# qope/starky-bn254

Measured on AMD Instinct MI355X. Metric: G1 scalar-mult proofs/sec at trace height 2^16, higher is better.
Workload: dtype u64

## Files before the change

starky_bn254_amd/csrc/kernels.cuh:

```cuda
#pragma once
#include "poseidon.cuh"
#include "air.cuh"

#include "kernels_ntt.cuh"

__global__ void pow_table_kernel(u64* out, size_t n, u64 base) {
  size_t i = (size_t)blockIdx.x * blockDim.x + threadIdx.x;
  if (i < n) out[i] = f_pow(F(base), i).v;
}
__global__ void shift_odd_table_kernel(u64* out, size_t n, const u64* __restrict__ shift, const u64* __restrict__ tw, u32 log_s) {
  size_t i = (size_t)blockIdx.x * blockDim.x + threadIdx.x;
  if (i < n) out[i] = (F(shift[i]) * F(tw[(i >> log_s) << log_s])).v;
}
__global__ void scale_pow_kernel(u64* v, size_t n, u64 base) {
  size_t i = (size_t)blockIdx.x * blockDim.x + threadIdx.x;
  if (i < n) v[i] = (F(v[i]) * f_pow(F(base), i)).v;
}

__global__ __launch_bounds__(256) __attribute__((amdgpu_waves_per_eu(4))) void leaf_hash_kernel(const u64* __restrict__ lde, size_t m, u32 lde_log, u32 ncols,
                                                        u64* __restrict__ digests) {
  size_t row = (size_t)blockIdx.x * blockDim.x + threadIdx.x;
  if (row >= m) return;
  F s[12];
#pragma unroll
  for (int i = 0; i < 12; i++) s[i] = F(0);
  size_t leaf = bitrev32((u32)row, lde_log);
  if (ncols <= 4) {
    for (u32 c = 0; c < 4; c++) digests[leaf * 4 + c] = c < ncols ? lde[(size_t)c * m + row] : 0;
    return;
  }
  for (u32 c = 0; c < ncols; c += 8) {
#pragma unroll
    for (u32 i = 0; i < 8; i++)
      if (c + i < ncols) s[i] = F(lde[(size_t)(c + i) * m + row]);
    poseidon_permute_keep(s, c + 8 >= ncols ? P_KEEP_DIGEST : (c + 16 <= ncols ? P_KEEP_CAPACITY : P_KEEP_ALL));
  }
#pragma unroll
  for (int i = 0; i < 4; i++) digests[leaf * 4 + i] = s[i].v;
}

__global__ __launch_bounds__(256) void merkle_level_kernel(const u64* __restrict__ child, u64* __restrict__ parent, size_t nparent) {
  size_t i = (size_t)blockIdx.x * blockDim.x + threadIdx.x;
  if (i >= nparent) return;
  F s[12];
#pragma unroll
  for (int k = 0; k < 8; k++) s[k] = F(child[i * 8 + k]);
#pragma unroll
  for (int k = 8; k < 12; k++) s[k] = F(0);
  poseidon_permute_keep(s, P_KEEP_DIGEST);
#pragma unroll
  for (int k = 0; k < 4; k++) parent[i * 4 + k] = s[k].v;
}

__global__ __launch_bounds__(256) __attribute__((amdgpu_waves_per_eu(4))) void leaf_absorb_kernel(const u64* __restrict__ lde_chunk, size_t m, u32 lde_log, u32 ncols_chunk,
                                                          u64* __restrict__ state, int first, int last, u64* __restrict__ digests, int next_full) {
  size_t row = (size_t)blockIdx.x * blockDim.x + threadIdx.x;
  if (row >= m) return;
  F s[12];
#pragma unroll
  for (int i = 0; i < 12; i++) s[i] = F(0);
  if (!first) {
#pragma unroll
    for (int i = 8; i < 12; i++) s[i] = F(state[(size_t)i * m + row]);
    if (ncols_chunk < 8) {
#pragma unroll
      for (int i = 0; i < 8; i++) s[i] = F(state[(size_t)i * m + row]);
    }
  }
  for (u32 c = 0; c < ncols_chunk; c += 8) {
#pragma unroll
    for (u32 i = 0; i < 8; i++)
      if (c + i < ncols_chunk) s[i] = F(lde_chunk[(size_t)(c + i) * m + row]);
    const bool end = c + 8 >= ncols_chunk;
    const int keep = end ? (last ? P_KEEP_DIGEST : (next_full ? P_KEEP_CAPACITY : P_KEEP_ALL)) : (c + 16 <= ncols_chunk ? P_KEEP_CAPACITY : P_KEEP_ALL);
    poseidon_permute_keep(s, keep);
  }
  u32 tid = threadIdx.x;
  asm volatile("" : "+v"(tid));
  const size_t row2 = (size_t)blockIdx.x * blockDim.x + tid;
  if (last) {
    size_t leaf = bitrev32((u32)row2, lde_log);
#pragma unroll
    for (int i = 0; i < 4; i++) digests[leaf * 4 + i] = s[i].v;
  } else {
#pragma unroll
    for (int i = 8; i < 12; i++) state[(size_t)i * m + row2] = s[i].v;
    if (!next_full) {
#pragma unroll
      for (int i = 0; i < 8; i++) state[(size_t)i * m + row2] = s[i].v;
    }
  }
}

static constexpr u32 MERKLE_SUBTREE_THREADS = 256;
__global__ __launch_bounds__(MERKLE_SUBTREE_THREADS) void merkle_subtree_kernel(u64* __restrict__ tree, size_t nleaf, u32 l0, u32 nlev, u32 nchild) {
  __shared__ u64 buf[2 * 256 * 4];
  const u32 tid = threadIdx.x, nt = blockDim.x;
  const u64* child = tree + (2 * nleaf - ((2 * nleaf) >> l0)) * 4;
  size_t base = (size_t)blockIdx.x * nchild;
  for (u32 e = tid; e < nchild * 4; e += nt) buf[e] = child[base * 4 + e];
  __syncthreads();
  u32 active = nchild / 2;
  const u32 groups = nt / 16, grp = tid / 16, lane = tid & 15;
  for (u32 lv = 1; lv <= nlev; lv++) {
    u64* out = tree + (2 * nleaf - ((2 * nleaf) >> (l0 + lv))) * 4;
    const size_t idx0 = ((size_t)blockIdx.x * nchild) >> lv;
    if (active > 4 * groups) {
      F s[12];
      if (tid < active) {
#pragma unroll
        for (int k = 0; k < 8; k++) s[k] = F(buf[tid * 8 + k]);
#pragma unroll
        for (int k = 8; k < 12; k++) s[k] = F(0);
        poseidon_permute_keep(s, P_KEEP_DIGEST);
      }
      __syncthreads();
      if (tid < active) {
#pragma unroll
        for (int k = 0; k < 4; k++) { buf[tid * 4 + k] = s[k].v; out[(idx0 + tid) * 4 + k] = s[k].v; }
      }
      __syncthreads();
    } else {
      u64 res[4];
      u32 nit = (active + groups - 1) / groups;
      for (u32 it = 0; it < nit; it++) {
        u32 parent = it * groups + grp;
        if (it * groups + (tid / 64) * 4 >= active) break;
        const u32 e = lane < 12 ? lane : lane - 12;
        u64 v = (parent < active && e < 8) ? buf[parent * 8 + e] : 0;
        res[it] = poseidon_permute_coop16(v, lane);
      }
      __syncthreads();
      for (u32 it = 0; it < nit; it++) {
        u32 parent = it * groups + grp;
        if (parent < active && lane < 4) { buf[parent * 4 + lane] = res[it]; out[(idx0 + parent) * 4 + lane] = res[it]; }
      }
      __syncthreads();
    }
    active >>= 1;
  }
}

__global__ __launch_bounds__(256) void merkle_level_thread_kernel(u64* __restrict__ tree, size_t nleaf, u32 l) {
  const size_t parents = nleaf >> (l + 1);
  const size_t i = (size_t)blockIdx.x * blockDim.x + threadIdx.x;
  if (i >= parents) return;
  const u64* child = tree + (2 * nleaf - ((2 * nleaf) >> l)) * 4;
  u64* out = tree + (2 * nleaf - ((2 * nleaf) >> (l + 1))) * 4;
  F s[12];
#pragma unroll
  for (int k = 0; k < 8; k++) s[k] = F(child[i * 8 + k]);
#pragma unroll
  for (int k = 8; k < 12; k++) s[k] = F(0);
  poseidon_permute_keep(s, P_KEEP_DIGEST);
#pragma unroll
  for (int k = 0; k < 4; k++) out[i * 4 + k] = s[k].v;
}
__global__ __launch_bounds__(256) void merkle_level_coop_kernel(u64* __restrict__ tree, size_t nleaf, u32 l) {
  const size_t parents = nleaf >> (l + 1);
  const size_t parent = ((size_t)blockIdx.x * blockDim.x + threadIdx.x) >> 4;
  const u32 lane = threadIdx.x & 15, e = lane < 12 ? lane : lane - 12;
  const u64* child = tree + (2 * nleaf - ((2 * nleaf) >> l)) * 4;
  u64* out = tree + (2 * nleaf - ((2 * nleaf) >> (l + 1))) * 4;
  const u64 v = (parent < parents && e < 8) ? child[parent * 8 + e] : 0;
  const u64 r = poseidon_permute_coop16(v, lane);
  if (parent < parents && lane < 4) out[parent * 4 + lane] = r;
}

__global__ __launch_bounds__(256) void fri_leaf_hash_kernel(const u64* __restrict__ va, const u64* __restrict__ vb, u32 log_m, u32 arity_bits,
// ... 202 lines not shown
  } else if (KIND == 11) {
    if (PART == 0) flag_u64_eval(cs, row, FlagU64Shape(p.num_io));
  } else if (KIND == 7 || KIND == 8) {
    const OpShape sh(KIND);
    if (PART == 0) op_eval<KIND>(cs, row, sh);
    else if (PART == 2) {
      if (seg == 2) permutation_checks(cs, row, zrow, sh, p.num_zs, F(p.gamma0), F(p.gamma1), 0, p.zsplit);
      else permutation_checks(cs, row, zrow, sh, p.num_zs, F(p.gamma0), F(p.gamma1), p.zsplit, p.num_zs);
    }
  } else {
    constexpr int E = KIND == 4 ? 12 : (KIND == 6 ? 13 : (KIND == 3 ? 2 : (KIND == 5 ? 0 : 1)));
    ExpShape sh(E, p.num_io);
    const bool moved = (E == 0 || E == 1 || E == 2) && p.lookups_in_perm;
    if (PART < 2) exp_eval<E>(cs, row, sh, (const ExpPiConsts<F>*)pic_arg, (PART == 1 && moved) ? 3 : 1 + PART);
    else {
      const int z0 = seg == 2 ? 0 : p.zsplit, z1 = seg == 2 ? p.zsplit : p.num_zs;
      permutation_checks(cs, row, zrow, sh, p.num_zs, F(p.gamma0), F(p.gamma1), z0, z1);
      if (moved) lookups_beside_permutation(cs, row, sh, p.num_zs, (z0 + 1) / 2, (z1 + 1) / 2);
    }
  }
#pragma unroll
  for (int j = 0; j < SBN_NCH; j++) p.part[((size_t)seg * SBN_NCH + j) * p.m + i] = cs.result(j).v;
}
__global__ __launch_bounds__(256) void quotient_combine_kernel(QuotientParams p) {
  size_t i = (size_t)blockIdx.x * blockDim.x + threadIdx.x;
  if (i >= p.m) return;
  F dinv(p.zh_inv[((i << p.row_shift) | p.row_rho) & 1]);
#pragma unroll
  for (int j = 0; j < SBN_NCH; j++) {
    F acc(p.part[((size_t)(QSEG - 1) * SBN_NCH + j) * p.m + i]);
#pragma unroll
    for (u32 sgm = 0; sgm + 1 < QSEG; sgm++) acc += F(p.part[((size_t)sgm * SBN_NCH + j) * p.m + i]) * F(p.seg_shift[sgm][j]);
    p.qout[(size_t)j * p.m + i] = (acc * dinv).v;
  }
}

__global__ void domain_tables_kernel(u64* xs, u64* lag_first, u64* lag_last, size_t m, u32 lde_log, u32 degree_bits) {
  size_t i = (size_t)blockIdx.x * blockDim.x + threadIdx.x;
  if (i >= m) return;
  F w = f_root_of_unity(lde_log);
  F x = F(GL_GEN) * f_pow(w, i);
  F g = f_root_of_unity(degree_bits);
  F nn = F((u64)1 << degree_bits);
  F zx = f_exp_pow2(x, degree_bits) - F(1);
  xs[i] = x.v;
  lag_first[i] = (zx * f_inv(nn * (x - F(1)))).v;
  lag_last[i] = (zx * f_inv(nn * (g * x - F(1)))).v;
}

__device__ __forceinline__ F wave_scan_mul_rev(F x, int lane) {
#pragma unroll
  for (int d = 1; d < 64; d <<= 1) {
    u64 o = __shfl_down((unsigned long long)x.v, d, 64);
    if (lane + d < 64) x = x * F(o);
  }
  return x;
}
template <int PZ_E>
__global__ __launch_bounds__(256) void permz_chunk_products_kernel(const u64* __restrict__ trace, size_t n, const PairCols* __restrict__ pairs, u64 gamma0, u64 gamma1,
                                                                   u64* __restrict__ tot) {
  __shared__ u64 wn[4], wd[4];
  const int z = blockIdx.y;
  const size_t c = blockIdx.x, chunks = gridDim.x;
  const int tid = threadIdx.x, lane = tid & 63, wv = tid >> 6;
  const size_t i0 = c * 256 * PZ_E + (size_t)tid * PZ_E;
  const u64* lhs = trace + (size_t)pairs[z].lhs * n + i0;
  const u64* rhs = trace + (size_t)pairs[z].rhs * n + i0;
  const F g0(gamma0), g1(gamma1);
  u64 lv[PZ_E], rv[PZ_E];
#pragma unroll
  for (int e = 0; e < PZ_E; e++) { lv[e] = lhs[e]; rv[e] = rhs[e]; }
  F pn(1), pd(1);
#pragma unroll
  for (int e = 0; e < PZ_E; e++) { const F l(lv[e]), r(rv[e]); pn = pn * ((l + g0) * (l + g1)); pd = pd * ((r + g0) * (r + g1)); }
#pragma unroll
  for (int d = 32; d >= 1; d >>= 1) { pn = pn * F(__shfl_xor((unsigned long long)pn.v, d, 64)); pd = pd * F(__shfl_xor((unsigned long long)pd.v, d, 64)); }
  if (lane == 0) { wn[wv] = pn.v; wd[wv] = pd.v; }
  __syncthreads();
  if (tid == 0) {
    tot[((size_t)z * chunks + c) * 2] = (F(wn[0]) * F(wn[1]) * F(wn[2]) * F(wn[3])).v;
    tot[((size_t)z * chunks + c) * 2 + 1] = (F(wd[0]) * F(wd[1]) * F(wd[2]) * F(wd[3])).v;
  }
}
__global__ __launch_bounds__(64) void permz_chunk_scan_kernel(const u64* __restrict__ tot, u32 chunks, u64* __restrict__ pq) {
  const int z = blockIdx.x, lane = threadIdx.x;
  const u64* t = tot + (size_t)z * chunks * 2;
  u64* o = pq + (size_t)z * chunks * 2;
  F carry(1), all(1);
  for (u32 b = 0; b < chunks; b += 64) {
    const u32 idx = b + lane;
    const bool on = idx < chunks;
    const F inc = wave_scan_mul(on ? F(t[2 * idx]) : F(1), lane);
    const u64 pv = __shfl_up((unsigned long long)inc.v, 1, 64);
    if (on) o[2 * idx] = (lane == 0 ? carry : carry * F(pv)).v;
    carry = carry * F(__shfl((unsigned long long)inc.v, 63, 64));
    F d = on ? F(t[2 * idx + 1]) : F(1);
#pragma unroll
    for (int k = 32; k >= 1; k >>= 1) d = d * F(__shfl_xor((unsigned long long)d.v, k, 64));
    all = all * d;
  }
  F carry_s = f_inv(all);
  for (u32 b = ((chunks - 1) / 64) * 64;; b -= 64) {
    const u32 idx = b + lane;
    const bool on = idx < chunks;
    const F inc = wave_scan_mul_rev(on ? F(t[2 * idx + 1]) : F(1), lane);
    const u64 sv = __shfl_down((unsigned long long)inc.v, 1, 64);
    if (on) o[2 * idx + 1] = (lane == 63 ? carry_s : carry_s * F(sv)).v;
    carry_s = carry_s * F(__shfl((unsigned long long)inc.v, 0, 64));
    if (b == 0) break;
  }
}
template <int PZ_E>
__global__ __launch_bounds__(256) void permz_chunk_write_kernel(const u64* __restrict__ trace, size_t n, const PairCols* __restrict__ pairs, u64 gamma0, u64 gamma1,
                                                                const u64* __restrict__ pq, u64* __restrict__ zout) {
  __shared__ u64 wn[4], wd[4];
  const int z = blockIdx.y;
  const size_t c = blockIdx.x, chunks = gridDim.x;
  const int tid = threadIdx.x, lane = tid & 63, wv = tid >> 6;
  const size_t i0 = c * 256 * PZ_E + (size_t)tid * PZ_E;
  const u64* lhs = trace + (size_t)pairs[z].lhs * n + i0;
  const u64* rhs = trace + (size_t)pairs[z].rhs * n + i0;
  u64* zc = zout + (size_t)z * n + i0;
  const F g0(gamma0), g1(gamma1);
  u64 lv[PZ_E], rv[PZ_E];
#pragma unroll
  for (int e = 0; e < PZ_E; e++) { lv[e] = lhs[e]; rv[e] = rhs[e]; }
  F pn[PZ_E], sd[PZ_E];
#pragma unroll
  for (int e = 0; e < PZ_E; e++) { const F l(lv[e]); const F num = (l + g0) * (l + g1); pn[e] = e ? pn[e - 1] * num : num; }
#pragma unroll
  for (int e = PZ_E - 1; e >= 0; e--) { const F r(rv[e]); const F den = (r + g0) * (r + g1); sd[e] = e < PZ_E - 1 ? sd[e + 1] * den : den; }
  const F incn = wave_scan_mul(pn[PZ_E - 1], lane), incd = wave_scan_mul_rev(sd[0], lane);
  if (lane == 63) wn[wv] = incn.v;
  if (lane == 0) wd[wv] = incd.v;
  __syncthreads();
  F pre(pq[((size_t)z * chunks + c) * 2]), suf(pq[((size_t)z * chunks + c) * 2 + 1]);
  for (int w = 0; w < wv; w++) pre = pre * F(wn[w]);
  for (int w = 3; w > wv; w--) suf = suf * F(wd[w]);
  const u64 pv = __shfl_up((unsigned long long)incn.v, 1, 64), sv = __shfl_down((unsigned long long)incd.v, 1, 64);
  const F exn = lane == 0 ? pre : pre * F(pv);
  const F exd = lane == 63 ? suf : suf * F(sv);
  const F both = exn * exd;
  zc[0] = (both * sd[0]).v;
#pragma unroll
  for (int e = 1; e < PZ_E; e++) zc[e] = (both * pn[e - 1] * sd[e]).v;
}

__global__ void ext_pow_table_kernel(u64* pa, u64* pb, size_t n, u64 z0, u64 z1) {
  size_t i = (size_t)blockIdx.x * blockDim.x + threadIdx.x;
  if (i >= n) return;
  E2 r = e2_pow(E2(F(z0), F(z1)), i);
  pa[i] = r.a.v; pb[i] = r.b.v;
}
__device__ __forceinline__ F block_sum(F v, u64* sh) {
  const int lane = threadIdx.x & 63, wv = threadIdx.x >> 6;
#pragma unroll
  for (int d = 32; d >= 1; d >>= 1) v = v + F(__shfl_xor((unsigned long long)v.v, d, 64));
  __syncthreads();
  if (lane == 0) sh[wv] = v.v;
  __syncthreads();
  F t(0);
  for (unsigned w = 0; w < blockDim.x / 64; w++) t = t + F(sh[w]);
  return t;
}
template <u32 OPEN_UNROLL>
__global__ __launch_bounds__(256) void openings_kernel(const u64* __restrict__ coeffs, size_t n, const u64* __restrict__ pa0, const u64* __restrict__ pb0,
                                                       const u64* __restrict__ pa1, const u64* __restrict__ pb1, u64* __restrict__ out) {
  __shared__ u64 sh[4];
  const u64* c = coeffs + (size_t)blockIdx.x * n;
  Acc<F> s0, r0, s1, r1;
  s0.clear(); r0.clear(); s1.clear(); r1.clear();
  for (size_t i = threadIdx.x; i < n; i += 256 * OPEN_UNROLL) {
    u64 cv[OPEN_UNROLL], t0[OPEN_UNROLL], t1[OPEN_UNROLL], t2[OPEN_UNROLL], t3[OPEN_UNROLL];
#pragma unroll
    for (u32 k = 0; k < OPEN_UNROLL; k++) {
      const size_t ik = i + 256 * k;
      cv[k] = c[ik]; t0[k] = pa0[ik]; t1[k] = pb0[ik]; t2[k] = pa1[ik]; t3[k] = pb1[ik];
    }
    __builtin_amdgcn_sched_barrier(0);
#pragma unroll
    for (u32 k = 0; k < OPEN_UNROLL; k++) {
      const F v{cv[k]};
      s0.macv(v, F(t0[k])); r0.macv(v, F(t1[k]));
      s1.macv(v, F(t2[k])); r1.macv(v, F(t3[k]));
    }
  }
  const F a0 = block_sum(s0.value(), sh), b0 = block_sum(r0.value(), sh), a1 = block_sum(s1.value(), sh), b1 = block_sum(r1.value(), sh);
  if (threadIdx.x == 0) {
    u64* o = out + (size_t)blockIdx.x * 4;
    o[0] = a0.v; o[1] = b0.v; o[2] = a1.v; o[3] = b1.v;
  }
}

template <u32 OPEN_UNROLL>
__global__ __launch_bounds__(256) void openings1_kernel(const u64* __restrict__ coeffs, size_t n, const u64* __restrict__ pa, const u64* __restrict__ pb,
                                                        u64* __restrict__ out, u32 off) {
  __shared__ u64 sh[4];
  const u64* c = coeffs + (size_t)blockIdx.x * n;
  Acc<F> s0, r0;
  s0.clear(); r0.clear();
  for (size_t i = threadIdx.x; i < n; i += 256 * OPEN_UNROLL) {
    u64 cv[OPEN_UNROLL], t0[OPEN_UNROLL], t1[OPEN_UNROLL];
#pragma unroll
    for (u32 k = 0; k < OPEN_UNROLL; k++) {
      const size_t ik = i + 256 * k;
      cv[k] = c[ik]; t0[k] = pa[ik]; t1[k] = pb[ik];
    }
    __builtin_amdgcn_sched_barrier(0);
#pragma unroll
    for (u32 k = 0; k < OPEN_UNROLL; k++) {
      const F v{cv[k]};
      s0.macv(v, F(t0[k])); r0.macv(v, F(t1[k]));
    }
  }
  const F a0 = block_sum(s0.value(), sh), b0 = block_sum(r0.value(), sh);
  if (threadIdx.x == 0) {
    u64* o = out + (size_t)blockIdx.x * 4 + off;
    o[0] = a0.v; o[1] = b0.v;
  }
}

__global__ __launch_bounds__(256) void fri_combine_partial_kernel(const u64* __restrict__ coeffs, size_t n, u32 npoly, u32 group_size,
                                                                  const u64* __restrict__ pa, const u64* __restrict__ pb, u64* __restrict__ part_a,
                                                                  u64* __restrict__ part_b) {
  size_t i = (size_t)blockIdx.x * blockDim.x + threadIdx.x;
  if (i >= n) return;
  const u32 g = blockIdx.y;
  const u32 j0 = g * group_size, cnt = j0 + group_size < npoly ? group_size : npoly - j0;
  const u64* c = coeffs + (size_t)j0 * n + i;
  Acc<F> a, b;
  a.clear(); b.clear();
  u32 k = 0;
  for (; k + 8 <= cnt; k += 8) {
    u64 f[8];
#pragma unroll
    for (u32 u = 0; u < 8; u++) f[u] = c[(size_t)(k + u) * n];
#pragma unroll
    for (u32 u = 0; u < 8; u++) { const F v(f[u]); a.mac(v, F(pa[k + u])); b.mac(v, F(pb[k + u])); }
  }
  for (; k < cnt; k++) { const F v(c[(size_t)k * n]); a.mac(v, F(pa[k])); b.mac(v, F(pb[k])); }
  part_a[(size_t)g * n + i] = a.value().v; part_b[(size_t)g * n + i] = b.value().v;
}
__global__ void fri_combine_reduce_kernel(const u64* part_a, const u64* part_b, size_t n, u32 ngroups, const u64* w, u64* out_a, u64* out_b, int accumulate) {
  size_t i = (size_t)blockIdx.x * blockDim.x + threadIdx.x;
  if (i >= n) return;
  E2 acc = accumulate ? E2(F(out_a[i]), F(out_b[i])) : E2(F(0), F(0));
  for (u32 g = 0; g < ngroups; g++) acc += E2(F(part_a[(size_t)g * n + i]), F(part_b[(size_t)g * n + i])) * E2(F(w[2 * g]), F(w[2 * g + 1]));
  out_a[i] = acc.a.v; out_b[i] = acc.b.v;
}

static constexpr u32 DBL_CHUNK = 16;
__global__ __launch_bounds__(256) void divide_by_linear_pass1(const u64* __restrict__ ca, const u64* __restrict__ cb, size_t nchunks, u64 z0, u64 z1,
                                                              u64* __restrict__ ha, u64* __restrict__ hb) {
  const size_t t = (size_t)blockIdx.x * blockDim.x + threadIdx.x;
  if (t >= nchunks) return;
  const E2 z{F(z0), F(z1)};
  const size_t s = t * DBL_CHUNK;
  E2 h{F(0), F(0)};
  for (u32 k = DBL_CHUNK; k-- > 0;) h = h * z + E2(F(ca[s + k]), F(cb[s + k]));
  ha[t] = h.a.v; hb[t] = h.b.v;
}
template <u32 U> __device__ __forceinline__ void dbl_fold(const u64* ha, const u64* hb, size_t base, size_t per, const E2 zl, E2& g) {
  for (size_t j0 = per; j0 > 0; j0 -= U) {
    u64 va[U], vb[U];
#pragma unroll
    for (u32 k = 0; k < U; k++) { va[k] = ha[base + j0 - 1 - k]; vb[k] = hb[base + j0 - 1 - k]; }
#pragma unroll
    for (u32 k = 0; k < U; k++) g = E2(F(va[k]), F(vb[k])) + zl * g;
  }
}
template <u32 U> __device__ __forceinline__ void dbl_replay(u64* ha, u64* hb, size_t base, size_t per, const E2 zl, E2 carry) {
  for (size_t j0 = per; j0 > 0; j0 -= U) {
    u64 va[U], vb[U];
#pragma unroll
    for (u32 k = 0; k < U; k++) { va[k] = ha[base + j0 - 1 - k]; vb[k] = hb[base + j0 - 1 - k]; }
#pragma unroll
    for (u32 k = 0; k < U; k++) {
      ha[base + j0 - 1 - k] = carry.a.v; hb[base + j0 - 1 - k] = carry.b.v;
      carry = E2(F(va[k]), F(vb[k])) + zl * carry;
    }
  }
}
__global__ __launch_bounds__(256) void divide_by_linear_pass2(u64* __restrict__ ha, u64* __restrict__ hb, size_t nchunks, u64 z0, u64 z1) {
  __shared__ u64 sa[2][256], sb[2][256];
  const int tid = threadIdx.x;
  const int lanes = nchunks < 256 ? (int)nchunks : 256;
  const size_t per = nchunks / lanes, base = (size_t)tid * per;
  const bool live = tid < lanes;
  const E2 zl = e2_pow(E2{F(z0), F(z1)}, DBL_CHUNK);
  E2 g{F(0), F(0)};
  if (live) { if (per % 8 == 0) dbl_fold<8>(ha, hb, base, per, zl, g); else dbl_fold<1>(ha, hb, base, per, zl, g); }
  E2 m = e2_pow(zl, per);
  int cur = 0;
  sa[0][tid] = g.a.v; sb[0][tid] = g.b.v;
  __syncthreads();
  for (int d = 1; d < lanes; d <<= 1) {
    E2 v{F(sa[cur][tid]), F(sb[cur][tid])};
    if (tid + d < lanes) v = v + m * E2(F(sa[cur][tid + d]), F(sb[cur][tid + d]));
    sa[cur ^ 1][tid] = v.a.v; sb[cur ^ 1][tid] = v.b.v;
    m = m * m;
    cur ^= 1;
    __syncthreads();
  }
  E2 carry{F(0), F(0)};
  if (tid + 1 < lanes) carry = E2(F(sa[cur][tid + 1]), F(sb[cur][tid + 1]));
  if (live) { if (per % 8 == 0) dbl_replay<8>(ha, hb, base, per, zl, carry); else dbl_replay<1>(ha, hb, base, per, zl, carry); }
}
__global__ __launch_bounds__(256) void divide_by_linear_pass3(const u64* __restrict__ ca, const u64* __restrict__ cb, size_t nchunks, u64 z0, u64 z1,
                                                              const u64* __restrict__ ha, const u64* __restrict__ hb, u64 mul0, u64 mul1,
                                                              u64* __restrict__ oa, u64* __restrict__ ob, int accumulate, u32 times_x) {
  const size_t t = (size_t)blockIdx.x * blockDim.x + threadIdx.x;
  if (t >= nchunks) return;
  const E2 z{F(z0), F(z1)}, mul{F(mul0), F(mul1)};
  const size_t s = t * DBL_CHUNK, n = nchunks * DBL_CHUNK;
  E2 b{F(ha[t]), F(hb[t])};
  for (u32 k = DBL_CHUNK; k-- > 0;) {
    const size_t i = s + k;
    const E2 q = b;
    b = b * z + E2(F(ca[i]), F(cb[i]));
    const size_t j = i + times_x;
    if (j >= n) continue;
    const E2 o = accumulate ? E2(F(oa[j]), F(ob[j])) * mul + q : q;
    oa[j] = o.a.v; ob[j] = o.b.v;
  }
}

__global__ void fri_fold_kernel(const u64* ca, const u64* cb, size_t nout, u32 arity, u64 b0, u64 b1, u64* oa, u64* ob) {
  size_t i = (size_t)blockIdx.x * blockDim.x + threadIdx.x;
  if (i >= nout) return;
  E2 beta{F(b0), F(b1)}, acc(F(0), F(0));
  for (u32 t = arity; t-- > 0;) acc = acc * beta + E2(F(ca[i * arity + t]), F(cb[i * arity + t]));
  oa[i] = acc.a.v; ob[i] = acc.b.v;
}

struct PowParams { u64 state[12]; u32 wpos; u32 min_lz; u64 base; u64 count; u64* result; };
__global__ __launch_bounds__(256) void pow_kernel(PowParams p) {
  u64 gid = (u64)blockIdx.x * blockDim.x + threadIdx.x;
  if (gid >= p.count) return;
  F s[12];
#pragma unroll
  for (int i = 0; i < 12; i++) s[i] = F(p.state[i]);
  s[p.wpos] = F(p.base + gid);
  poseidon_permute(s);
  u64 resp = s[P_RATE - 1].v;
  u32 lz = resp ? (u32)__clzll((long long)resp) : 64;
  if (lz >= p.min_lz) atomicMin((unsigned long long*)p.result, (unsigned long long)(p.base + gid));
}

__global__ __launch_bounds__(256) void split_pack_kernel(const u64* __restrict__ lde, size_t m, u32 nc, u32 ob, u32 log_r, u32 me,
                                                         u64* __restrict__ send_l, u64* __restrict__ send_n, u64* __restrict__ self_l, u64* __restrict__ self_n) {
  const size_t i = (size_t)blockIdx.x * blockDim.x + threadIdx.x;
  const u32 c = blockIdx.y;
  if (i >= m || c >= nc) return;
  const u64 v = lde[(size_t)c * m + i];
  const size_t ml = m >> log_r, rmask = ((size_t)1 << log_r) - 1;
  const u32 s = bitrev32((u32)(i & rmask), log_r);
  if (s == me) self_l[(size_t)c * ml + (i >> log_r)] = v;
  else send_l[((size_t)s * ob + c) * ml + (i >> log_r)] = v;
  if (send_n) {
    const size_t p = (i + m - 2) & (m - 1);
    const u32 s2 = bitrev32((u32)(p & rmask), log_r);
    if (s2 == me) self_n[(size_t)c * ml + (p >> log_r)] = v;
    else send_n[((size_t)s2 * ob + c) * ml + (p >> log_r)] = v;
  }
}
__global__ void split_unpack_rows_kernel(const u64* __restrict__ in, size_t m, u32 nplanes, u32 log_r, u64* __restrict__ out) {
  const size_t i = (size_t)blockIdx.x * blockDim.x + threadIdx.x;
  if (i >= m) return;
  const size_t ml = m >> log_r;
  const u32 s = bitrev32((u32)(i & (((size_t)1 << log_r) - 1)), log_r);
  for (u32 p = 0; p < nplanes; p++) out[(size_t)p * m + i] = in[((size_t)s * nplanes + p) * ml + (i >> log_r)];
// ... 36 lines not shown
```

starky_bn254_amd/csrc/poseidon.cuh:

```cuda
#pragma once
#include "gl.cuh"
#include "settings.hpp"
#include <utility>

static constexpr int P_WIDTH = 12;
static constexpr int P_RATE = 8;
enum { P_KEEP_ALL = 0, P_KEEP_CAPACITY = 1, P_KEEP_DIGEST = 2 };

static const u64 POSEIDON_RC_HOST[360] = {
#include "poseidon_consts.inc"
};
static __constant__ u64 POSEIDON_RC_DEV[360] = {
#include "poseidon_consts.inc"
};

static const u64 POSEIDON_EFF_HOST[360] = {
#include "poseidon_eff_consts.inc"
};
static __constant__ u64 POSEIDON_EFF_DEV[360] = {
#include "poseidon_eff_consts.inc"
};

static __constant__ u64 POSEIDON_KX_DEV[8 * 24] = {
#include "poseidon_kx_consts.inc"
// ... 226 lines not shown
}
__device__ __forceinline__ void mds3(u64* s, u64 d1, u64 d2, u64 tb) {
  u32 lo[12], hi[12];
#pragma unroll
  for (int i = 0; i < 12; i++) { lo[i] = (u32)s[i]; hi[i] = (u32)(s[i] >> 32); }
  u64 al[12], ah[12];
  mds3_half(lo, (u32)d1, (u32)d2, al, tb);
  mds3_half(hi, (u32)(d1 >> 32), (u32)(d2 >> 32), ah, tb);
#pragma unroll
  for (int r = 0; r < 12; r += 3) fold3(al + r, ah + r, s + r);
}
}

__device__ __forceinline__ void poseidon_permute_fast(F* st, int keep = P_KEEP_ALL) {
  u64 rcb = (u64)POSEIDON_EFF_DEV, tb = (u64)pw::MDS_FUSED_TABLE, kxb = (u64)POSEIDON_KX_DEV;
  asm volatile("" : "+s"(rcb), "+s"(tb), "+s"(kxb));
  typedef const __attribute__((address_space(4))) u64* cptr;
  const cptr rc = (cptr)rcb;
  const pw::kx_ptr kx = (pw::kx_ptr)kxb;
  u64 s[12];
#pragma unroll
  for (int i = 0; i < 12; i++) s[i] = pw::add_c(st[i].v, rc[i]);
  int r = 4;
#pragma unroll 1
  for (int k = 0; k < 4; k++) {
    u32 lo[12], hi[12];
#pragma unroll
    for (int i = 0; i < 12; i += 3) pw::sbox3(s[i], s[i + 1], s[i + 2], lo + i, hi + i);
    pw::mdsc(lo, hi, s, kx + 24 * k);
  }
#pragma unroll 1
  for (int k = 0; k < 6; k++, r += 3) {
    s[0] = pw::sbox(pw::add_c(s[0], rc[12 * r]));
    const u64 y0p = pw::sbox(pw::add_c(pw::mds_row0(s), rc[12 * (r + 1)]));
    const u64 z0p = pw::sbox(pw::add_c(pw::mds2_row0(s, y0p, tb), rc[12 * (r + 2)]));
    pw::mds3(s, y0p, z0p, tb);
  }
#pragma unroll 1
  for (int k = 0; k < 2; k++, r += 2) {
    s[0] = pw::sbox(pw::add_c(s[0], rc[12 * r]));
    pw::mds2(s, pw::sbox(pw::add_c(pw::mds_row0(s), rc[12 * (r + 1)])), tb);
  }
#pragma unroll
  for (int i = 0; i < 12; i++) s[i] = pw::add_c(s[i], rc[12 * 26 + i]);
#pragma unroll 1
  for (int k = 4; k < 7; k++) {
    u32 lo[12], hi[12];
#pragma unroll
    for (int i = 0; i < 12; i += 3) pw::sbox3(s[i], s[i + 1], s[i + 2], lo + i, hi + i);
    pw::mdsc(lo, hi, s, kx + 24 * k);
  }
  {
    u32 lo[12], hi[12];
#pragma unroll
    for (int i = 0; i < 12; i += 3) pw::sbox3(s[i], s[i + 1], s[i + 2], lo + i, hi + i);
    if (keep == P_KEEP_CAPACITY) {
      pw::mdsq<8>(lo, hi, s + 8);
#pragma unroll
      for (int i = 8; i < 12; i++) st[i] = F(gp::canon(s[i]));
    } else if (keep == P_KEEP_DIGEST) {
      pw::mdsq<0>(lo, hi, s);
#pragma unroll
      for (int i = 0; i < 4; i++) st[i] = F(gp::canon(s[i]));
    } else {
      pw::mds(lo, hi, s);
#pragma unroll
      for (int i = 0; i < 12; i++) st[i] = F(gp::canon(s[i]));
    }
  }
}
namespace pc {
template <int I> __device__ __forceinline__ u32 rot(u32 x, bool use2) {
  const u32 y1 = (u32)__builtin_amdgcn_update_dpp(0, (int)x, 0x120 + (16 - I), 0xf, 0xf, false);
  const u32 y2 = (u32)__builtin_amdgcn_update_dpp(0, (int)x, 0x120 + (12 - I), 0xf, 0xf, false);
  return use2 ? y2 : y1;
}
template <int I> __device__ __forceinline__ void term(u32 lo, u32 hi, u32 lane16, u64& al, u64& ah) {
  constexpr u32 C[12] = {17, 15, 41, 16, 2, 28, 13, 13, 39, 18, 34, 20};
  if constexpr (I == 0) { al += (u64)lo * C[0]; ah += (u64)hi * C[0]; }
  else {
    const bool use2 = lane16 >= 12 || lane16 + I >= 16;
    al += (u64)rot<I>(lo, use2) * C[I]; ah += (u64)rot<I>(hi, use2) * C[I];
  }
}
template <int... I> __device__ __forceinline__ void mds_row(u32 lo, u32 hi, u32 lane16, u64& al, u64& ah, std::integer_sequence<int, I...>) {
  (term<I>(lo, hi, lane16, al, ah), ...);
}
}
__device__ __forceinline__ u64 poseidon_permute_coop16(u64 v, u32 lane) {
  const u64* rc = POSEIDON_EFF_DEV;
  const u32 lane16 = lane & 15, j = lane16 < 12 ? lane16 : lane16 - 12;
  for (int r = 0; r < 30; r++) {
    v = pw::add_c(v, rc[12 * r + j]);
    const bool full = r < 4 || r >= 26;
    u64 sb = pw::sbox(v);
    v = (full || j == 0) ? sb : v;
    u32 lo = (u32)v, hi = (u32)(v >> 32);
    u64 al = 0, ah = 0;
    pc::mds_row(lo, hi, lane16, al, ah, std::make_integer_sequence<int, 12>{});
    if (j == 0) { al += (u64)lo * 8u; ah += (u64)hi * 8u; }
    u32 h0 = (u32)ah, h1 = (u32)(ah >> 32);
    u64 t = al + ((u64)h0 << 32);
    u32 c = t < al;
    u64 add = (u64)(h1 + c) * GLEPS;
    u64 o = t + add;
    if (o < add) o += GLEPS;
    v = o;
  }
  return v >= GLP ? v - GLP : v;
}
#else
__device__ u64 poseidon_permute_coop16(u64 v, u32 lane);
#endif

#if !defined(__HIP_DEVICE_COMPILE__)
#include "poseidon_fast_consts.inc"
namespace ph {
typedef unsigned __int128 u128;
struct Acc { u128 lo = 0, hi = 0; };
static inline void mac(Acc& a, u64 x, u64 y) { u128 p = (u128)x * y; a.lo += (u64)p; a.hi += (u64)(p >> 64); }
static inline u64 fold(const Acc& a) {
  u128 t = a.lo + a.hi * (u128)GLEPS;
  return gl_reduce128((u64)t, (u64)(t >> 64));
}
}
#if defined(__x86_64__)
#include <immintrin.h>
#include <cstdlib>
#define PH_AVX512 __attribute__((target("avx512f,avx512dq")))
PH_AVX512 static inline __m512i mulred_x8(__m512i a, __m512i b) {
  const __m512i M32 = _mm512_set1_epi64(0xFFFFFFFFLL);
  const __m512i ah = _mm512_srli_epi64(a, 32), bh = _mm512_srli_epi64(b, 32);
  const __m512i ll = _mm512_mul_epu32(a, b), lh = _mm512_mul_epu32(a, bh), hl = _mm512_mul_epu32(ah, b), hh = _mm512_mul_epu32(ah, bh);
  const __m512i mid = _mm512_add_epi64(lh, _mm512_srli_epi64(ll, 32));
  const __m512i mid2 = _mm512_add_epi64(hl, _mm512_and_si512(mid, M32));
  const __m512i lo = _mm512_or_si512(_mm512_and_si512(ll, M32), _mm512_slli_epi64(mid2, 32));
  const __m512i hi = _mm512_add_epi64(hh, _mm512_add_epi64(_mm512_srli_epi64(mid, 32), _mm512_srli_epi64(mid2, 32)));
  const __m512i hi_hi = _mm512_srli_epi64(hi, 32), hi_lo = _mm512_and_si512(hi, M32);
  const __mmask8 bw = _mm512_cmplt_epu64_mask(lo, hi_hi);
  __m512i t0 = _mm512_sub_epi64(lo, hi_hi);
  t0 = _mm512_mask_sub_epi64(t0, bw, t0, M32);
  const __m512i t1 = _mm512_sub_epi64(_mm512_slli_epi64(hi_lo, 32), hi_lo);
  __m512i r = _mm512_add_epi64(t0, t1);
  const __mmask8 cy = _mm512_cmplt_epu64_mask(r, t1);
  return _mm512_mask_add_epi64(r, cy, r, M32);
}
PH_AVX512 static inline __m512i sbox7_x8(__m512i x, __m512i c) {
  const __m512i M32 = _mm512_set1_epi64(0xFFFFFFFFLL);
  __m512i y = _mm512_add_epi64(x, c);
  y = _mm512_mask_add_epi64(y, _mm512_cmplt_epu64_mask(y, c), y, M32);
  const __m512i y2 = mulred_x8(y, y), y4 = mulred_x8(y2, y2), y3 = mulred_x8(y2, y);
  return mulred_x8(y4, y3);
}
PH_AVX512 static void full_round_sboxes_avx512(u64* s, const u64* rc) {
  const __m512i a = sbox7_x8(_mm512_loadu_si512(s), _mm512_loadu_si512(rc));
  const __m512i b = sbox7_x8(_mm512_maskz_loadu_epi64(0x0F, s + 8), _mm512_maskz_loadu_epi64(0x0F, rc + 8));
  _mm512_storeu_si512(s, a);
  _mm512_mask_storeu_epi64(s + 8, 0x0F, b);
}
PH_AVX512 static inline void mds_x12(__m512i& A, __m512i& B) {
  static const u64 C[12] = {17, 15, 41, 16, 2, 28, 13, 13, 39, 18, 34, 20};
  const __m512i M32 = _mm512_set1_epi64(0xFFFFFFFFLL);
  const __m512i lane = _mm512_set_epi64(7, 6, 5, 4, 3, 2, 1, 0);
  const __m512i twelve = _mm512_set1_epi64(12);
  __m512i slA = _mm512_setzero_si512(), shA = slA, slB = slA, shB = slA;
#pragma GCC unroll 12
  for (int i = 0; i < 12; i++) {
    __m512i ia = _mm512_add_epi64(lane, _mm512_set1_epi64(i));
    ia = _mm512_mask_sub_epi64(ia, _mm512_cmpge_epu64_mask(ia, twelve), ia, twelve);
    __m512i ib = _mm512_add_epi64(lane, _mm512_set1_epi64((i + 8) % 12));
    ib = _mm512_mask_sub_epi64(ib, _mm512_cmpge_epu64_mask(ib, twelve), ib, twelve);
    const __m512i xa = _mm512_permutex2var_epi64(A, ia, B), xb = _mm512_permutex2var_epi64(A, ib, B);
    const __m512i ca = i == 0 ? _mm512_set_epi64(17, 17, 17, 17, 17, 17, 17, 25) : _mm512_set1_epi64((long long)C[i]);
    const __m512i cb = _mm512_set1_epi64((long long)C[i]);
    slA = _mm512_add_epi64(slA, _mm512_mul_epu32(xa, ca)); shA = _mm512_add_epi64(shA, _mm512_mul_epu32(_mm512_srli_epi64(xa, 32), ca));
    slB = _mm512_add_epi64(slB, _mm512_mul_epu32(xb, cb)); shB = _mm512_add_epi64(shB, _mm512_mul_epu32(_mm512_srli_epi64(xb, 32), cb));
  }
  auto fold = [&](__m512i sl, __m512i sh) PH_AVX512 {
    const __m512i shl = _mm512_slli_epi64(sh, 32);
    const __m512i l = _mm512_add_epi64(sl, shl);
    const __m512i one = _mm512_set1_epi64(1);
    __m512i h = _mm512_srli_epi64(sh, 32);
    h = _mm512_mask_add_epi64(h, _mm512_cmplt_epu64_mask(l, shl), h, one);
    const __m512i t1 = _mm512_sub_epi64(_mm512_slli_epi64(h, 32), h);
    const __m512i r = _mm512_add_epi64(l, t1);
    return _mm512_mask_add_epi64(r, _mm512_cmplt_epu64_mask(r, t1), r, M32);
  };
  A = fold(slA, shA); B = fold(slB, shB);
}
PH_AVX512 static void full_rounds_x4_avx512(u64* s, const u64* rc) {
  __m512i A = _mm512_loadu_si512(s), B = _mm512_maskz_loadu_epi64(0x0F, s + 8);
  for (int k = 0; k < 4; k++) {
    A = sbox7_x8(A, _mm512_loadu_si512(rc + 12 * k));
    B = sbox7_x8(B, _mm512_maskz_loadu_epi64(0x0F, rc + 12 * k + 8));
    mds_x12(A, B);
  }
  const __m512i P = _mm512_set1_epi64((long long)GLP);
  A = _mm512_mask_sub_epi64(A, _mm512_cmpge_epu64_mask(A, P), A, P);
  B = _mm512_mask_sub_epi64(B, _mm512_cmpge_epu64_mask(B, P), B, P);
  _mm512_storeu_si512(s, A);
  _mm512_mask_storeu_epi64(s + 8, 0x0F, B);
}
static inline bool host_has_avx512() {
  static const bool have = __builtin_cpu_supports("avx512f") && __builtin_cpu_supports("avx512dq") && !sbn::Settings::from_env_or_default().no_avx512;
  return have;
}
#endif
static inline void full_rounds_host(F* s, const u64* rc, int& r) {
#if defined(__x86_64__)
  if (host_has_avx512()) {
    static_assert(sizeof(F) == sizeof(u64), "F is one u64");
    full_rounds_x4_avx512(reinterpret_cast<u64*>(s), rc + 12 * r);
    r += 4;
    return;
  }
#endif
  for (int k = 0; k < 4; k++, r++) {
    for (int i = 0; i < 12; i++) s[i] = sbox7(s[i] + F(rc[12 * r + i]));
    poseidon_mds(s);
  }
}
struct PartialChainTables { u64 PI[22][11]; u64 K[22][22]; };
static inline const PartialChainTables& partial_chain_tables() {
  static const PartialChainTables T = [] {
    PartialChainTables t{};
    for (int k = 0; k < 22; k++) {
      for (int j = 0; j < 11; j++) { F acc(0); for (int i = 0; i < 11; i++) acc = acc + F(PFAST_VHAT[11 * k + i]) * F(PFAST_INIT[11 * i + j]); t.PI[k][j] = acc.v; }
      for (int q = 0; q < k; q++) { F acc(0); for (int i = 0; i < 11; i++) acc = acc + F(PFAST_VHAT[11 * k + i]) * F(PFAST_WHAT[11 * q + i]); t.K[k][q] = acc.v; }
    }
    return t;
  }();
  return T;
}
static inline void poseidon_permute_host_fast(F* s) {
  const u64* rc = POSEIDON_EFF_HOST;
  int r = 0;
  full_rounds_host(s, rc, r);
  for (int i = 0; i < 12; i++) s[i] = s[i] + F(rc[12 * r + i]);
  const PartialChainTables& T = partial_chain_tables();
  u64 u[11], t[22];
  for (int i = 0; i < 11; i++) u[i] = s[1 + i].v;
  ph::Acc fin[11];
  for (int i = 0; i < 11; i++) for (int j = 0; j < 11; j++) ph::mac(fin[i], PFAST_INIT[11 * i + j], u[j]);
  ph::Acc nxt; for (int j = 0; j < 11; j++) ph::mac(nxt, T.PI[0][j], u[j]);
  u64 cur = s[0].v;
  for (int k = 0; k < 22; k++, r++) {
    t[k] = sbox7(k ? F(cur) + F(rc[12 * r]) : F(cur)).v;
    ph::Acc a = nxt;
    for (int q = 0; q < k; q++) ph::mac(a, T.K[k][q], t[q]);
    ph::mac(a, PFAST_M00, t[k]);
    cur = ph::fold(a);
    nxt = ph::Acc();
    if (k + 1 < 22) for (int j = 0; j < 11; j++) ph::mac(nxt, T.PI[k + 1][j], u[j]);
    for (int i = 0; i < 11; i++) ph::mac(fin[i], PFAST_WHAT[11 * k + i], t[k]);
  }
  s[0] = F(cur);
  for (int i = 0; i < 11; i++) s[1 + i] = F(ph::fold(fin[i]));
  full_rounds_host(s, rc, r);
}
#endif

GL_HD void poseidon_permute(F* s) {
#if defined(__HIP_DEVICE_COMPILE__)
  poseidon_permute_fast(s);
#else
  poseidon_permute_host_fast(s);
#endif
}
GL_HD void poseidon_permute_keep(F* s, int keep) {
#if defined(__HIP_DEVICE_COMPILE__)
  poseidon_permute_fast(s, keep);
#else
  (void)keep;
  poseidon_permute_host_fast(s);
#endif
}

struct Digest4 { F e[4]; };

GL_HD Digest4 poseidon_two_to_one(const Digest4& l, const Digest4& r) {
  F s[12];
#pragma unroll
  for (int i = 0; i < 4; i++) { s[i] = l.e[i]; s[4 + i] = r.e[i]; s[8 + i] = F(0); }
  poseidon_permute(s);
  Digest4 d;
#pragma unroll
  for (int i = 0; i < 4; i++) d.e[i] = s[i];
  return d;
}
```

starky_bn254_amd/csrc/prover.hip:

```cpp
#include "host_common.hpp"
#include "settings.hpp"
#include "kernels.cuh"
#include "kernels_tracegen.cuh"
#include <algorithm>
#include <cstring>
#include <cstdlib>
#include <thread>
#include <atomic>
#include <chrono>

using namespace sbn;

namespace sbn { thread_local std::string g_last_error; }

#define HIPC(expr)                                                                                   \
  do {                                                                                               \
    hipError_t e_ = (expr);                                                                          \
    if (e_ != hipSuccess) return fail(SBN_ERR_HIP, "%s failed: %s (%s:%d)", #expr, hipGetErrorString(e_), __FILE__, __LINE__); \
  } while (0)

static std::atomic<int> g_default_device{0};
static thread_local int t_device = -1;
static inline int cur_device() { return t_device >= 0 ? t_device : g_default_device.load(); }
#define g_device (cur_device())
namespace sbn { int current_device() { return cur_device(); } }

enum Stage {
  ST_TRACE_COMMIT, ST_PERM_Z, ST_Z_COMMIT, ST_QUOTIENT_EVAL, ST_QUOTIENT_COMMIT,
  ST_OPENINGS, ST_FRI_COMBINE, ST_FRI_LAYERS, ST_POW, ST_QUERIES, ST_COUNT
};
enum Extra { EX_TRACE_ABSORB_MS, EX_TRACE_ABSORB_LAUNCHES, EX_Z_ABSORB_MS, EX_Z_ABSORB_LAUNCHES, EX_TRACEGEN_MS, EX_COMM_MS, EX_COUNT };
static const char* STAGE_NAMES[ST_COUNT + EX_COUNT] = {
  "trace_commit", "perm_z", "z_commit", "quotient_eval", "quotient_commit",
  "openings", "fri_combine", "fri_layers", "pow", "queries",
  "trace_absorb_kernels_ms", "trace_absorb_launches", "z_absorb_kernels_ms", "z_absorb_launches", "device_tracegen_ms",
  "split_exchange_ms"};
static constexpr int MAX_CHUNKS = 512;

struct DevTree {
  u64* d = nullptr; size_t nleaf = 0; u32 nlevels = 0;
  u64* level(u32 l) const { return d + (2 * nleaf - ((2 * nleaf) >> l)) * 4; }
};

struct ColShare {
  size_t total = 0, ob = 64; u32 R = 1, rank = 0;
  size_t nblocks() const { return (total + ob - 1) / ob; }
  size_t steps() const { return (nblocks() + R - 1) / R; }
  size_t block_cols(size_t b) const { return b < nblocks() ? std::min(ob, total - b * ob) : 0; }
  size_t own_cols(u32 r) const { size_t s = 0; for (size_t b = r; b < nblocks(); b += R) s += block_cols(b); return s; }
  size_t own() const { return own_cols(rank); }
  size_t max_own() const { size_t s = 0; for (u32 r = 0; r < R; r++) s = std::max(s, own_cols(r)); return s; }
  size_t global_col(u32 r, size_t local) const { return ((local / ob) * R + r) * ob + local % ob; }
};
struct SplitCtx {
  sbn_comm comm;
  u32 log_r = 0, rho = 0;
  size_t ml = 0;
  ColShare cs, zs;
  size_t cr = 0, zr = 0;
  u32 planes = 1;
  u64 *lde_l = nullptr, *lde_n = nullptr, *zlde_l = nullptr, *zlde_n = nullptr, *scratch = nullptr;
  size_t scratch_words = 0;
  size_t slot_words = 0;
  u64* d_ldechunk = nullptr;
  u32* d_idx_local = nullptr;
  PairCols* d_pairs_own = nullptr;
  hipStream_t cstream = nullptr;
  hipEvent_t xchg_done[MAX_CHUNKS];
  std::vector<hipEvent_t> tev;
  size_t tev_used = 0;
};

struct sbn_prover {
  AirShape air; sbn_config cfg; FriShape fri;
  SplitCtx* sp = nullptr;
  size_t lde_scratch_words = 0;
  u32 degree_bits, lde_log; size_t n, m;
  int device; hipStream_t stream;
  u64 *d_trace = nullptr, *d_coef = nullptr, *d_lde = nullptr, *d_tmp = nullptr;
  u64 *d_zval = nullptr, *d_zcoef = nullptr, *d_zlde = nullptr;
  u64 *d_q = nullptr, *d_qlde = nullptr;
  DevTree tree_t, tree_z, tree_q;
  std::vector<DevTree> fri_trees;
  u64 *d_tw_f = nullptr, *d_tw_i = nullptr, *d_shift = nullptr, *d_shift_inv = nullptr;
  u64 *d_shift_odd = nullptr;
  u64 *d_xs = nullptr, *d_lag_first = nullptr, *d_lag_last = nullptr;
  u64 *d_apow = nullptr;
  size_t apow_n = 0;
  void* d_pic = nullptr;
  PairCols* d_pairs = nullptr;
  u64 *d_zpow = nullptr;
  u64 *d_open = nullptr;
  u64 *d_part = nullptr;
  u64 *d_w = nullptr;
  u64 *d_fa = nullptr, *d_fb = nullptr;
  u64 *d_fcoef = nullptr;
  u64 *d_fcoef2 = nullptr;
  std::vector<u64*> fri_vals;
  u64 *d_pow = nullptr;
  u32 *d_idx = nullptr;
  u64 *d_qbuf = nullptr; size_t qstride = 0;
  std::vector<u64> pi;
  bool loaded = false;
  hipEvent_t ev[ST_COUNT + 1];
  float stage_ms[ST_COUNT + EX_COUNT];
  size_t ntt_chunk;
  size_t ntt_sub = 0;
  bool ntt_xcd = true;
  bool fast_ntt = true;
  bool ntt_fused = false;
  u64* d_tmp2 = nullptr;
  hipStream_t rstream = nullptr;
  hipEvent_t rows_done = nullptr, rc_done = nullptr;
  int* d_rc_err = nullptr;
  bool rc_pending = false;
  size_t rc_first_col = 0;
  u64* d_tmp3 = nullptr;
  bool ntt_fused512 = false;
  hipStream_t hstream = nullptr;
  hipStream_t nstream = nullptr;
  hipEvent_t intt_done[MAX_CHUNKS];
  bool ntt_two_streams = false;
  Settings set;
  unsigned gen_calls = 0;
  int chain_mode = 0;
  hipEvent_t chunk_ready[MAX_CHUNKS];
  hipEvent_t abs_ev[2 * MAX_CHUNKS];
  hipEvent_t hash_done;
  u64* d_sponge = nullptr;
  u64* h_chain = nullptr;
  size_t h_chain_words = 0;
  u64* h_io = nullptr;
  size_t h_io_words = 0;
  u64* h_open = nullptr;
  u64* h_open2 = nullptr;
};

static int dmalloc(u64** p, size_t words) {
  HIPC(hipMalloc((void**)p, words * sizeof(u64)));
  return 0;
}

static u32 pick_log_t(u32 log_r, u32 log_s) {
  u32 lt = 4;
  while (lt > 0 && ((size_t)(1u << log_r) * ((1u << lt) + 1) * 8) > 48 * 1024) lt--;
  return std::min(lt, log_s);
}
static int ntt_columns(sbn_prover* P, const u64* in, size_t in_cs, u64* out, size_t out_cs, u64* tmp, size_t tmp_cs, size_t ncols,
                       u32 log_n, bool inverse, size_t n_in, const u64* pre, const u64* post, u64 scale, hipStream_t st = nullptr, int which = 3) {
  if (ncols == 0) return 0;
  if (!st) st = P->stream;
  u32 log_n1 = (log_n + 1) / 2, log_n2 = log_n - log_n1;
  size_t n1 = (size_t)1 << log_n1, n2 = (size_t)1 << log_n2;
  NttPassParams a{};
  a.in = in; a.out = tmp; a.in_col_stride = in_cs; a.out_col_stride = tmp_cs;
  a.log_r = log_n1; a.log_t = pick_log_t(log_n1, log_n2); a.log_n = log_n;
  a.in_sr = n2; a.in_st = 1; a.out_sr = n2; a.out_st = 1; a.n_in = n_in;
  a.r_fast_load = 0; a.twiddle = 1; a.tw = inverse ? P->d_tw_i : P->d_tw_f; a.tw_log = P->lde_log;
  a.pre = pre; a.post = nullptr; a.scale = 1;
  NttPassParams b{};
  b.in = tmp; b.out = out; b.in_col_stride = tmp_cs; b.out_col_stride = out_cs;
  b.log_r = log_n2; b.log_t = pick_log_t(log_n2, log_n1); b.log_n = log_n;
  b.in_sr = 1; b.in_st = n2; b.out_sr = n1; b.out_st = 1; b.n_in = (size_t)1 << log_n;
  b.r_fast_load = 1; b.twiddle = 0; b.tw = a.tw; b.tw_log = P->lde_log;
  b.pre = nullptr; b.post = post; b.scale = scale;
  for (size_t c0 = 0; c0 < ncols; c0 += 32768) {
    size_t nc = std::min<size_t>(32768, ncols - c0);
    NttPassParams pa = a, pb = b;
    pa.in = a.in + c0 * in_cs; pa.out = a.out + c0 * tmp_cs;
    pb.in = b.in + c0 * tmp_cs; pb.out = b.out + c0 * out_cs;
    dim3 ga((unsigned)(n2 >> pa.log_t), (unsigned)nc), gb((unsigned)(n1 >> pb.log_t), (unsigned)nc);
    size_t la = ((size_t)1 << pa.log_r) * ((1u << pa.log_t) + 1) * 8, lb = ((size_t)1 << pb.log_r) * ((1u << pb.log_t) + 1) * 8;
    const u32 kperm = inverse ? 11u : 5u;
    auto launch = [&](NttPassParams q, dim3 grid, size_t lds_bytes) {
      const bool fast = P->fast_ntt && q.log_t == 4 && (q.log_r == 8 || q.log_r == 9);
      if (fast && P->ntt_xcd) { q.xcd_order = 1; std::swap(grid.x, grid.y); }
      if (fast && q.log_r == 8) hipLaunchKernelGGL(ntt_fast_pass_kernel<0>, grid, dim3(256), 16 * 272 * 8, st, q, kperm);
      else if (fast) hipLaunchKernelGGL(ntt_fast_pass_kernel<1>, grid, dim3(256), 32 * 272 * 8, st, q, kperm);
      else hipLaunchKernelGGL(ntt_pass_kernel, grid, dim3(NTT_THREADS), lds_bytes, st, q);
    };
    if (P->fast_ntt && pa.log_r == 9 && log_n2 >= 4) pa.log_t = 4;
    if (P->fast_ntt && pb.log_r == 9 && log_n1 >= 4) pb.log_t = 4;
    const bool split_a = P->fast_ntt && !inverse && pa.log_r == 10 && log_n2 >= 4 && pa.in_st == 1 && n_in <= (size_t)512 * pa.in_sr && pre == P->d_shift && P->d_shift_odd;
    if (split_a) { pa.log_r = 9; pa.log_t = 4; pa.split = 1; pa.pre2 = P->d_shift_odd; }
    ga = dim3((unsigned)(n2 >> pa.log_t), (unsigned)nc, split_a ? 2u : 1u); gb = dim3((unsigned)(n1 >> pb.log_t), (unsigned)nc);
    la = ((size_t)1 << pa.log_r) * ((1u << pa.log_t) + 1) * 8; lb = ((size_t)1 << pb.log_r) * ((1u << pb.log_t) + 1) * 8;
    if (which & 1) launch(pa, ga, la);
    if (which & 2) launch(pb, gb, lb);
  }
  HIPC(hipGetLastError());
  return 0;
}

static u64 host_inv_pow2(u32 k) { return f_inv(F((u64)1 << k)).v; }
static constexpr int SBN_MAX_DEVICES = 64;
static int ntt_fast_setup() {
  static std::atomic<bool> done[SBN_MAX_DEVICES];
  const int d = g_device >= 0 && g_device < SBN_MAX_DEVICES ? g_device : 0;
  if (!done[d].load()) {
    HIPC(hipFuncSetAttribute((const void*)ntt_fast_pass_kernel<1>, hipFuncAttributeMaxDynamicSharedMemorySize, 32 * 272 * 8));
    HIPC(hipFuncSetAttribute((const void*)ntt_fused_inv_b_lde_a_kernel, hipFuncAttributeMaxDynamicSharedMemorySize, 32 * 272 * 8));
    HIPC(hipFuncSetAttribute((const void*)ntt_fused512_inv_b_lde_a_kernel, hipFuncAttributeMaxDynamicSharedMemorySize, 32 * 272 * 8));
    done[d].store(true);
  }
  return 0;
}

static int intt_values(sbn_prover* P, const u64* vals, u64* coef, size_t ncols) {
  for (size_t c0 = 0; c0 < ncols; c0 += P->ntt_chunk) {
    size_t nc = std::min(P->ntt_chunk, ncols - c0);
    int rc = ntt_columns(P, vals + c0 * P->n, P->n, coef + c0 * P->n, P->n, P->d_tmp, P->m, nc, P->degree_bits, true, P->n, nullptr, nullptr,
                         host_inv_pow2(P->degree_bits));
    if (rc) return rc;
  }
  return 0;
}
static int lde_coeffs(sbn_prover* P, const u64* coef, u64* lde, size_t ncols) {
  for (size_t c0 = 0; c0 < ncols; c0 += P->ntt_chunk) {
    size_t nc = std::min(P->ntt_chunk, ncols - c0);
    int rc = ntt_columns(P, coef + c0 * P->n, P->n, lde + c0 * P->m, P->m, P->d_tmp, P->m, nc, P->lde_log, false, P->n, P->d_shift, nullptr, 1);
    if (rc) return rc;
  }
  return 0;
}
static int intt_then_lde(sbn_prover* P, const u64* vals, u64* coef, u64* lde, size_t ncols) {
  for (size_t c0 = 0; c0 < ncols; c0 += P->ntt_chunk) {
    size_t nc = std::min(P->ntt_chunk, ncols - c0);
    int rc = ntt_columns(P, vals + c0 * P->n, P->n, coef + c0 * P->n, P->n, P->d_tmp, P->m, nc, P->degree_bits, true, P->n, nullptr, nullptr,
                         host_inv_pow2(P->degree_bits));
    if (rc) return rc;
    rc = ntt_columns(P, coef + c0 * P->n, P->n, lde + c0 * P->m, P->m, P->d_tmp, P->m, nc, P->lde_log, false, P->n, P->d_shift, nullptr, 1);
    if (rc) return rc;
  }
  return 0;
}

static int intt_lde_cols_fused(sbn_prover* P, const u64* v, u64* cf, u64* lde_out, size_t nc, u64* tmp2, hipStream_t lde_stream, hipEvent_t handoff) {
  int rc = ntt_columns(P, v, P->n, cf, P->n, P->d_tmp, P->m, nc, P->degree_bits, true, P->n, nullptr, nullptr, host_inv_pow2(P->degree_bits), nullptr, 1);
  if (rc) return rc;
  NttFusedParams f{};
  const u32 log_n1 = (P->degree_bits + 1) / 2;
  f.in = P->d_tmp; f.in_col_stride = P->m; f.coef = cf; f.coef_col_stride = P->n; f.out = tmp2; f.out_col_stride = P->m;
  f.n1 = (size_t)1 << log_n1; f.log_n = P->degree_bits; f.tw_i = P->d_tw_i; f.tw_f = P->d_tw_f; f.tw_log = P->lde_log; f.pre = P->d_shift; f.pre2 = P->d_shift_odd;
  f.scale = host_inv_pow2(P->degree_bits);
  if (P->ntt_fused512) hipLaunchKernelGGL(ntt_fused512_inv_b_lde_a_kernel, dim3((unsigned)nc, 32u), dim3(256), 32 * 272 * 8, P->stream, f);
  else hipLaunchKernelGGL(ntt_fused_inv_b_lde_a_kernel, dim3((unsigned)nc, (unsigned)(f.n1 >> 4)), dim3(256), 32 * 272 * 8, P->stream, f);
  if (lde_stream != P->stream) {
    HIPC(hipEventRecord(handoff, P->stream));
    HIPC(hipStreamWaitEvent(lde_stream, handoff, 0));
  }
  return ntt_columns(P, cf, P->n, lde_out, P->m, tmp2, P->m, nc, P->lde_log, false, P->n, P->d_shift, nullptr, 1, lde_stream, 2);
}
static int intt_lde_cols(sbn_prover* P, const u64* v, u64* cf, u64* lde_out, size_t nc) {
  if ((P->ntt_fused || P->ntt_fused512) && P->d_tmp2) return intt_lde_cols_fused(P, v, cf, lde_out, nc, P->d_tmp2, P->stream, nullptr);
  int rc = ntt_columns(P, v, P->n, cf, P->n, P->d_tmp, P->m, nc, P->degree_bits, true, P->n, nullptr, nullptr, host_inv_pow2(P->degree_bits));
  if (rc) return rc;
  return ntt_columns(P, cf, P->n, lde_out, P->m, P->d_tmp, P->m, nc, P->lde_log, false, P->n, P->d_shift, nullptr, 1);
}
static int intt_then_lde_chunk(sbn_prover* P, const u64* vals, u64* coef, u64* lde, size_t c0, size_t nc) {
  if (!P->ntt_sub) return intt_lde_cols(P, vals + c0 * P->n, coef + c0 * P->n, lde + c0 * P->m, nc);
  const size_t sub = P->ntt_sub ? P->ntt_sub : nc;
  for (size_t s0 = 0; s0 < nc; s0 += sub) {
    const size_t a = c0 + s0, k = std::min(sub, nc - s0);
    int rc = ntt_columns(P, vals + a * P->n, P->n, coef + a * P->n, P->n, P->d_tmp, P->m, k, P->degree_bits, true, P->n, nullptr, nullptr,
                         host_inv_pow2(P->degree_bits));
    if (rc) return rc;
    rc = ntt_columns(P, coef + a * P->n, P->n, lde + a * P->m, P->m, P->d_tmp, P->m, k, P->lde_log, false, P->n, P->d_shift, nullptr, 1);
    if (rc) return rc;
  }
  return 0;
}

static int tree_alloc(DevTree& t, size_t nleaf, u32 cap_height) {
  t.nleaf = nleaf;
  u32 lg = 0; while (((size_t)1 << lg) < nleaf) lg++;
  t.nlevels = lg - cap_height;
  return dmalloc(&t.d, 2 * nleaf * 4);
}
static int tree_build_inner(sbn_prover* P, DevTree& t, hipStream_t st) {
  const bool fuse = P->set.merkle_fuse;
  u32 l0 = 0;
  while (l0 < t.nlevels) {
    const size_t parents = t.nleaf >> (l0 + 1);
    if (fuse && parents <= 8192 && parents >= 16 && ((t.nleaf >> l0) % 32) == 0) {
      const u32 nlev = std::min<u32>(t.nlevels - l0, 5);
      hipLaunchKernelGGL(merkle_subtree_kernel, dim3((unsigned)((t.nleaf >> l0) / 32)), dim3(MERKLE_SUBTREE_THREADS), 0, st, t.d, t.nleaf, l0, nlev, 32u);
      l0 += nlev;
      continue;
// ... 73 lines not shown
  (void)ex_ms;
  return 0;
}
static thread_local double t_wait_deadline_s = 0;
static inline void poll_backoff(unsigned spins) {
  if (spins < 2000) std::this_thread::yield();
  else std::this_thread::sleep_for(std::chrono::microseconds(spins < 20000 ? 20 : 200));
}
static inline hipError_t stream_wait(hipStream_t st) {
  if (t_wait_deadline_s <= 0) return hipStreamSynchronize(st);
  const auto t0 = std::chrono::steady_clock::now();
  unsigned spins = 0;
  for (;;) {
    const hipError_t e = hipStreamQuery(st);
    if (e != hipErrorNotReady) return e;
    if (std::chrono::duration<double>(std::chrono::steady_clock::now() - t0).count() > t_wait_deadline_s) return hipErrorNotReady;
    poll_backoff(++spins);
  }
}
static inline hipError_t event_wait(hipEvent_t ev) {
  if (t_wait_deadline_s <= 0) return hipEventSynchronize(ev);
  const auto t0 = std::chrono::steady_clock::now();
  unsigned spins = 0;
  for (;;) {
    const hipError_t e = hipEventQuery(ev);
    if (e != hipErrorNotReady) return e;
    if (std::chrono::duration<double>(std::chrono::steady_clock::now() - t0).count() > t_wait_deadline_s) return hipErrorNotReady;
    poll_backoff(++spins);
  }
}
static int split_exchange(sbn_prover* P, hipStream_t st, const std::vector<uint64_t>& so, const std::vector<uint64_t>& sl, const std::vector<uint64_t>& ro,
                          const std::vector<uint64_t>& rl) {
  SplitCtx* S = P->sp;
  bool any = false;
  for (u32 r = 0; r < S->comm.world; r++) any = any || sl[r] || rl[r];
  if (!any) return 0;
  const bool timed = S->tev_used + 2 <= S->tev.size();
  if (timed) HIPC(hipEventRecord(S->tev[S->tev_used], st));
  const int rc = S->comm.all_to_all(S->comm.ctx, (void*)st, so.data(), sl.data(), ro.data(), rl.data());
  if (rc) return fail(SBN_ERR_HIP, "sbn_comm.all_to_all failed (%d)", rc);
  if (timed) { HIPC(hipEventRecord(S->tev[S->tev_used + 1], st)); S->tev_used += 2; }
  return 0;
}
static int split_all_gather_host(sbn_prover* P, const void* send, void* recv, size_t bytes) {
  SplitCtx* S = P->sp;
  const int rc = S->comm.all_gather_host(S->comm.ctx, send, recv, bytes);
  if (rc) return fail(SBN_ERR_HIP, "sbn_comm.all_gather_host failed (%d)", rc);
  return 0;
}
static int split_all_gather_device(sbn_prover* P, size_t words) {
  SplitCtx* S = P->sp;
  const u32 R = S->comm.world;
  if (words * R > S->scratch_words || words * sizeof(u64) > S->comm.send_bytes) return fail(SBN_ERR_HIP, "internal: split scratch too small");
  const uint64_t base = (uint64_t)((const char*)S->scratch - (const char*)S->comm.recv_buf);
  std::vector<uint64_t> so(R, 0), sl(R, words * sizeof(u64)), ro(R), rl(R, words * sizeof(u64));
  for (u32 r = 0; r < R; r++) ro[r] = base + (uint64_t)r * words * sizeof(u64);
  return split_exchange(P, P->stream, so, sl, ro, rl);
}
static int commit_split(sbn_prover* P, const ColShare& sh, const u64* vals, bool vals_global, u64* coef_own, u64* plane_l, u64* plane_n, DevTree& t) {
  SplitCtx* S = P->sp;
  const u32 R = S->comm.world, me = S->comm.rank;
  const size_t n = P->n, m = P->m, ml = S->ml, ob = sh.ob;
  const size_t steps = sh.steps();
  if (steps > (size_t)MAX_CHUNKS) return fail(SBN_ERR_UNSUPPORTED, "too many column blocks");
  const char* rbase = (const char*)S->comm.recv_buf;
  const char* sbase = (const char*)S->comm.send_buf;
  const u32 row_log = P->lde_log - S->log_r;
  for (size_t k = 0; k < steps; k++) {
    const size_t b = k * R + me, nc = sh.block_cols(b);
    hipStream_t tstream = P->stream;
    u64* const slot = (u64*)S->comm.send_buf + (k & 1) * S->slot_words;
    u64* const slot_n = S->planes == 2 ? slot + (size_t)R * ob * ml : nullptr;
    if (nc) {
      const u64* v = vals + (vals_global ? b : k) * ob * n;
      u64* cf = coef_own + k * ob * n;
      u64* lde_out = R == 1 ? plane_l + b * ob * m : S->d_ldechunk;
      const bool fused = P->ntt_fused || P->ntt_fused512;
      const bool two = P->ntt_two_streams && P->d_tmp2 && (!fused || P->d_tmp3);
      tstream = two ? P->nstream : P->stream;
      int rc;
      if (two && fused) {
        if (k >= 2) HIPC(hipStreamWaitEvent(P->stream, P->chunk_ready[k - 2], 0));
        rc = intt_lde_cols_fused(P, v, cf, lde_out, nc, (k & 1) ? P->d_tmp3 : P->d_tmp2, P->nstream, P->intt_done[k]);
      } else if (two) {
        rc = ntt_columns(P, v, n, cf, n, P->d_tmp, m, nc, P->degree_bits, true, n, nullptr, nullptr, host_inv_pow2(P->degree_bits));
        if (rc) return rc;
        HIPC(hipEventRecord(P->intt_done[k], P->stream));
        HIPC(hipStreamWaitEvent(P->nstream, P->intt_done[k], 0));
        rc = ntt_columns(P, cf, n, lde_out, m, P->d_tmp2, m, nc, P->lde_log, false, n, P->d_shift, nullptr, 1, P->nstream);
      } else rc = intt_lde_cols(P, v, cf, lde_out, nc);
      if (rc) return rc;
      if (R > 1 && k >= 2) HIPC(hipStreamWaitEvent(tstream, S->xchg_done[k - 2], 0));
      if (R > 1)
        hipLaunchKernelGGL(split_pack_kernel, dim3((unsigned)((m + 255) / 256), (unsigned)nc), dim3(256), 0, tstream, S->d_ldechunk, m, (u32)nc, (u32)ob, S->log_r, me,
                           slot, slot_n, plane_l + b * ob * ml, plane_n ? plane_n + b * ob * ml : nullptr);
      HIPC(hipGetLastError());
    }
    HIPC(hipEventRecord(P->chunk_ready[k], tstream));
    hipEvent_t arrived = P->chunk_ready[k];
    if (R > 1) {
      HIPC(hipStreamWaitEvent(S->cstream, P->chunk_ready[k], 0));
      for (u32 pl = 0; pl < S->planes; pl++) {
        const u64* dst = pl ? plane_n : plane_l;
        std::vector<uint64_t> so(R, 0), sl(R, 0), ro(R, 0), rl(R, 0);
        for (u32 r = 0; r < R; r++) {
          if (r == me) continue;
          so[r] = (uint64_t)((const char*)(slot + ((size_t)pl * R + r) * ob * ml) - sbase);
          sl[r] = (uint64_t)(nc * ml * sizeof(u64));
          const size_t br = k * R + r;
          ro[r] = (uint64_t)((const char*)(dst + br * ob * ml) - rbase);
          rl[r] = (uint64_t)(sh.block_cols(br) * ml * sizeof(u64));
        }
        int rc = split_exchange(P, S->cstream, so, sl, ro, rl);
        if (rc) return rc;
      }
      HIPC(hipEventRecord(S->xchg_done[k], S->cstream));
      arrived = S->xchg_done[k];
    }
    HIPC(hipStreamWaitEvent(P->hstream, arrived, 0));
    const size_t c_begin = k * R * ob, c_end = std::min(sh.total, (k + 1) * R * ob);
    for (size_t c0 = c_begin; c0 < c_end; c0 += ob) {
      const size_t ncs = std::min(ob, c_end - c0);
      hipLaunchKernelGGL(leaf_absorb_kernel, dim3((unsigned)((ml + 255) / 256)), dim3(256), 0, P->hstream, plane_l + c0 * ml, ml, row_log, (u32)ncs,
                         P->d_sponge, c0 == 0 ? 1 : 0, c0 + ncs == sh.total ? 1 : 0, t.d,
                         (c0 + ncs < sh.total && sh.total - (c0 + ncs) >= 8) ? 1 : 0);
    }
    HIPC(hipGetLastError());
  }
  int rc = tree_build_inner(P, t, P->hstream);
  if (rc) return rc;
  HIPC(hipEventRecord(P->hash_done, P->hstream));
  HIPC(hipStreamWaitEvent(P->stream, P->hash_done, 0));
  return 0;
}
static int split_cap_to_host(sbn_prover* P, const DevTree& t, std::vector<u64>& cap) {
  SplitCtx* S = P->sp;
  const size_t capn = (size_t)1 << P->cfg.cap_height, own = capn >> S->log_r;
  std::vector<u64> mine(own * 4);
  HIPC(hipMemcpyAsync(mine.data(), t.level(t.nlevels), own * 4 * sizeof(u64), hipMemcpyDeviceToHost, P->stream));
  HIPC(stream_wait(P->stream));
  cap.resize(capn * 4);
  return split_all_gather_host(P, mine.data(), cap.data(), own * 4 * sizeof(u64));
}
static int absorb_times(sbn_prover* P, size_t ncols, int ex_ms) {
  size_t nchunks = (ncols + P->ntt_chunk - 1) / P->ntt_chunk;
  float tot = 0;
  for (size_t k = 0; k < nchunks; k++) { float ms = 0; HIPC(hipEventElapsedTime(&ms, P->abs_ev[2 * k], P->abs_ev[2 * k + 1])); tot += ms; }
  P->stage_ms[ST_COUNT + ex_ms] = tot;
  return 0;
}
static int tree_cap_to_host(sbn_prover* P, const DevTree& t, std::vector<u64>& cap) {
  size_t capn = (size_t)1 << P->cfg.cap_height;
  cap.resize(capn * 4);
  HIPC(hipMemcpyAsync(cap.data(), t.level(t.nlevels), capn * 4 * sizeof(u64), hipMemcpyDeviceToHost, P->stream));
  HIPC(stream_wait(P->stream));
  return 0;
}

static constexpr size_t SPLIT_BLOCK = 64;
static int split_sizes(const AirShape& as, u32 degree_bits, u32 rate_bits, u32 world, size_t ob, uint64_t* send_bytes, uint64_t* recv_bytes, size_t* scratch_words,
                       size_t* slot_words) {
  const size_t n = (size_t)1 << degree_bits, m = n << rate_bits;
  const u32 planes = world >= 4 ? 2 : 1;
  const size_t sw = std::max<size_t>(2 * m, 2 * n * world);
  const size_t slot = world > 1 ? (size_t)planes * ob * m : 0;
  *send_bytes = (uint64_t)(std::max(std::max(2 * slot, 2 * (m / world)), 2 * n) * sizeof(u64));
  *recv_bytes = (uint64_t)(((as.ncols + as.nzs) * (m / world) * planes + sw) * sizeof(u64));
  *scratch_words = sw;
  if (slot_words) *slot_words = slot;
  return 0;
}
static int create_ctx(const sbn_air_desc* air, const sbn_config* cfg, uint32_t degree_bits, const sbn_comm* comm, sbn_prover** out);
extern "C" int sbn_prover_create(const sbn_air_desc* air, const sbn_config* cfg, uint32_t degree_bits, sbn_prover** out) {
  return create_ctx(air, cfg, degree_bits, nullptr, out);
}
static int create_ctx(const sbn_air_desc* air, const sbn_config* cfg, uint32_t degree_bits, const sbn_comm* comm, sbn_prover** out) {
  if (!air || !cfg || !out) return fail(SBN_ERR_BAD_ARG, "null argument");
  *out = nullptr;
  if (!config_supported(cfg)) return fail(SBN_ERR_UNSUPPORTED, "unsupported StarkConfig (need num_challenges=2, rate_bits=1)");
  AirShape as;
  if (!air_shape(air, cfg, as)) return fail(SBN_ERR_BAD_ARG, "unknown air kind / num_io");
  if (degree_bits < 9 || degree_bits > 22) return fail(SBN_ERR_UNSUPPORTED, "degree_bits out of range");
  if (as.kind == SBN_AIR_FLAGS && (512 * (size_t)as.num_io) != ((size_t)1 << degree_bits)) return fail(SBN_ERR_BAD_ARG, "FlagStark needs 512*num_io rows");
  if (as.kind == SBN_AIR_FLAGS_U64 && (128 * (size_t)as.num_io) != ((size_t)1 << degree_bits)) return fail(SBN_ERR_BAD_ARG, "the u64 FlagStark needs 128*num_io rows");
  if (is_exp_air(as.kind)) {
    if ((exp_rows_per_instance(as.kind) * as.num_io) != ((size_t)1 << degree_bits)) return fail(SBN_ERR_BAD_ARG, "the Exp tables need 512*num_io rows (FQ12_EXP_U64: 128*num_io)");
    if (as.kind != SBN_AIR_FQ12_EXP && as.kind != SBN_AIR_FQ12_EXP_U64 && degree_bits < 16)
      return fail(SBN_ERR_UNSUPPORTED, "G1_EXP / G2_EXP / FQ_EXP need >= 2^16 rows (u16 range check, range_check.rs:26)");
  }
  int ndev = 0;
  if (hipGetDeviceCount(&ndev) != hipSuccess || ndev == 0) return fail(SBN_ERR_NO_DEVICE, "no HIP device available: the prover path has no CPU fallback");
  HIPC(hipSetDevice(g_device));
  sbn_prover* P = new sbn_prover();
  P->air = as; P->cfg = *cfg; P->degree_bits = degree_bits; P->lde_log = degree_bits + cfg->rate_bits;
  P->n = (size_t)1 << degree_bits; P->m = (size_t)1 << P->lde_log;
  P->fri = fri_shape(*cfg, degree_bits);
  P->device = g_device;
  int rc = 0;
  auto acc = [&](int r) { if (!rc) rc = r; };
  auto hipc = [&](hipError_t e, const char* what) { if (e != hipSuccess && !rc) rc = fail(SBN_ERR_HIP, "%s failed: %s", what, hipGetErrorString(e)); };
  if (P->fri.total_arity() > degree_bits + cfg->rate_bits - cfg->cap_height) { sbn_prover_destroy(P); return fail(SBN_ERR_UNSUPPORTED, "FRI total reduction arity is too large"); }
  P->ntt_chunk = P->lde_log >= 18 ? 48 : 64;
  {
    std::string serr;
    if (!P->set.load(serr)) { sbn_prover_destroy(P); return fail(SBN_ERR_BAD_ARG, "%s", serr.c_str()); }
  }
  const Settings& set = P->set;
  if (set.ntt_chunk) P->ntt_chunk = (size_t)set.ntt_chunk;
  P->fast_ntt = set.fast_ntt; P->ntt_xcd = set.ntt_xcd;
  P->ntt_fused = P->fast_ntt && (degree_bits == 16 || degree_bits == 17) && set.ntt_fused;
  P->ntt_fused512 = P->fast_ntt && degree_bits == 18 && P->lde_log == 19 && set.ntt_split1024 && set.ntt_fused;
  if (P->ntt_fused512 && !set.ntt_chunk) P->ntt_chunk = 40;
  P->ntt_sub = (size_t)set.ntt_sub;
  P->chain_mode = set.device_chain >= 0 ? set.device_chain : ((tracegen_host_chains_vectorized() || tracegen_host_threads() >= 8) ? 0 : 2);
  acc(ntt_fast_setup());
  hipc(hipStreamCreate(&P->stream), "hipStreamCreate");
  hipc(hipStreamCreate(&P->hstream), "hipStreamCreate");
  if (is_exp_air(as.kind)) {
    hipc(hipStreamCreate(&P->rstream), "hipStreamCreate");
    hipc(hipEventCreateWithFlags(&P->rows_done, hipEventDisableTiming), "hipEventCreate");
    hipc(hipEventCreateWithFlags(&P->rc_done, hipEventDisableTiming), "hipEventCreate");
    hipc(hipMalloc((void**)&P->d_rc_err, 256), "hipMalloc");
  }
  P->ntt_two_streams = set.ntt_streams ? set.ntt_streams == 2 : P->lde_log >= 19;
  if (P->ntt_two_streams) {
    hipc(hipStreamCreate(&P->nstream), "hipStreamCreate");
    for (auto& e : P->intt_done) hipc(hipEventCreateWithFlags(&e, hipEventDisableTiming), "hipEventCreate");
  }
  for (auto& e : P->ev) hipc(hipEventCreate(&e), "hipEventCreate");
  for (auto& e : P->abs_ev) hipc(hipEventCreate(&e), "hipEventCreate");
  for (auto& e : P->chunk_ready) hipc(hipEventCreateWithFlags(&e, hipEventDisableTiming), "hipEventCreate");
  hipc(hipEventCreateWithFlags(&P->hash_done, hipEventDisableTiming), "hipEventCreate");
  for (auto& v : P->stage_ms) v = 0;
  if (rc) { sbn_prover_destroy(P); return rc; }
  const size_t n = P->n, m = P->m, C = as.ncols, Z = as.nzs;
  if (comm && (C <= 4 || Z == 0)) { sbn_prover_destroy(P); return fail(SBN_ERR_UNSUPPORTED, "the split prover covers the wide tables (this one has %zu columns and %zu permutation Zs)", C, Z); }
  if (comm) {
    const u32 R = comm->world;
    u32 lr = 0; while ((1u << lr) < R) lr++;
    uint64_t sb = 0, rb = 0; size_t sw = 0, slotw = 0;
    if (comm->struct_size != sizeof(sbn_comm)) { sbn_prover_destroy(P); return fail(SBN_ERR_BAD_ARG, "sbn_comm.struct_size does not match this library (ABI %d)", SBN_ABI_VERSION); }
    if (!set.ntt_chunk) P->ntt_chunk = SPLIT_BLOCK;
    if (P->ntt_chunk != SPLIT_BLOCK) { sbn_prover_destroy(P); return fail(SBN_ERR_UNSUPPORTED, "the split prover deals columns in blocks of %zu: unset SBN_NTT_CHUNK", SPLIT_BLOCK); }
    split_sizes(as, degree_bits, cfg->rate_bits, R, SPLIT_BLOCK, &sb, &rb, &sw, &slotw);
    if ((1u << lr) != R || lr > cfg->cap_height || comm->rank >= R || !comm->all_to_all || !comm->all_gather_host || !comm->send_buf || !comm->recv_buf ||
        comm->send_bytes < sb || comm->recv_bytes < rb) {
      sbn_prover_destroy(P);
      return fail(SBN_ERR_BAD_ARG, "bad sbn_comm (world must be a power of two <= 2^cap_height; staging buffers of sbn_split_exchange_bytes)");
    }
    for (const void* buf : {(const void*)comm->send_buf, (const void*)comm->recv_buf}) {
      hipPointerAttribute_t pa{};
      if (hipPointerGetAttributes(&pa, buf) != hipSuccess || pa.device != P->device) {
        (void)hipGetLastError();
        sbn_prover_destroy(P);
        return fail(SBN_ERR_BAD_ARG, "sbn_comm staging buffers do not live on this prover's device %d (call sbn_set_device before creating the transport)", g_device);
      }
    }
    SplitCtx* S = P->sp = new SplitCtx();
    for (auto& e : S->xchg_done) e = nullptr;
    S->comm = *comm; S->log_r = lr; S->rho = bitrev32(comm->rank, lr); S->ml = m >> lr; S->planes = R >= 4 ? 2 : 1;
    S->slot_words = slotw;
    S->cs.total = C; S->cs.ob = SPLIT_BLOCK; S->cs.R = R; S->cs.rank = comm->rank;
    S->zs = S->cs; S->zs.total = Z;
    S->cr = S->cs.own(); S->zr = S->zs.own();
    hipc(hipStreamCreate(&S->cstream), "hipStreamCreate");
    for (auto& e : S->xchg_done) hipc(hipEventCreateWithFlags(&e, hipEventDisableTiming), "hipEventCreate");
    S->tev.assign(2 * (2 * (S->cs.steps() + S->zs.steps()) + 8), nullptr);
    for (auto& e : S->tev) hipc(hipEventCreate(&e), "hipEventCreate");
    u64* rbuf = (u64*)comm->recv_buf;
    S->lde_l = rbuf; rbuf += C * S->ml;
    if (S->planes == 2) { S->lde_n = rbuf; rbuf += C * S->ml; }
    S->zlde_l = rbuf; rbuf += Z * S->ml;
    if (S->planes == 2) { S->zlde_n = rbuf; rbuf += Z * S->ml; }
    S->scratch = rbuf; S->scratch_words = sw;
    P->lde_scratch_words = (size_t)(rb / sizeof(u64));
    acc(dmalloc(&P->d_trace, C * n)); acc(dmalloc(&P->d_coef, std::max<size_t>(S->cr, 1) * n));
    acc(dmalloc(&P->d_zval, std::max<size_t>(S->zr, 1) * n)); acc(dmalloc(&P->d_zcoef, std::max<size_t>(S->zr, 1) * n));
    acc(dmalloc(&S->d_ldechunk, P->ntt_chunk * m));
    hipc(hipMalloc((void**)&S->d_idx_local, cfg->num_query_rounds * sizeof(u32)), "hipMalloc");
    acc(tree_alloc(P->tree_t, S->ml, cfg->cap_height - lr)); acc(tree_alloc(P->tree_z, S->ml, cfg->cap_height - lr));
  } else {
    P->lde_scratch_words = C * m;
    acc(dmalloc(&P->d_trace, C * n)); acc(dmalloc(&P->d_coef, C * n)); acc(dmalloc(&P->d_lde, C * m));
    acc(dmalloc(&P->d_zval, std::max<size_t>(Z, 1) * n)); acc(dmalloc(&P->d_zcoef, std::max<size_t>(Z, 1) * n)); acc(dmalloc(&P->d_zlde, std::max<size_t>(Z, 1) * m));
    acc(tree_alloc(P->tree_t, m, cfg->cap_height)); acc(tree_alloc(P->tree_z, m, cfg->cap_height));
  }
  acc(dmalloc(&P->d_tmp, std::max(P->ntt_chunk, (size_t)4) * m));
  if (P->ntt_fused || P->ntt_fused512 || P->ntt_two_streams) acc(dmalloc(&P->d_tmp2, std::max(P->ntt_chunk, (size_t)4) * m));
  if ((P->ntt_fused || P->ntt_fused512) && P->ntt_two_streams) acc(dmalloc(&P->d_tmp3, std::max(P->ntt_chunk, (size_t)4) * m));
  acc(dmalloc(&P->d_q, 2 * m)); acc(dmalloc(&P->d_qlde, 4 * m));
  acc(tree_alloc(P->tree_q, m, cfg->cap_height));
  acc(dmalloc(&P->d_tw_f, m)); acc(dmalloc(&P->d_tw_i, m)); acc(dmalloc(&P->d_shift, m)); acc(dmalloc(&P->d_shift_inv, m));
  if (P->lde_log == 19 && set.ntt_split1024) acc(dmalloc(&P->d_shift_odd, n));
  acc(dmalloc(&P->d_xs, m)); acc(dmalloc(&P->d_lag_first, m)); acc(dmalloc(&P->d_lag_last, m));
  P->apow_n = apow_len(as.nconstraints, as.nzs);
  acc(dmalloc(&P->d_apow, (size_t)SBN_NCH * P->apow_n));
  acc(dmalloc(&P->d_zpow, 4 * n)); acc(dmalloc(&P->d_open, (C + Z + 4) * 4));
  hipc(hipHostMalloc((void**)&P->h_open, (C + Z + 4) * 4 * sizeof(u64), hipHostMallocDefault), "hipHostMalloc");
  hipc(hipHostMalloc((void**)&P->h_open2, (C + Z) * 4 * sizeof(u64), hipHostMallocDefault), "hipHostMalloc");
  acc(dmalloc(&P->d_part, 2 * 32 * n)); acc(dmalloc(&P->d_w, 4096)); acc(dmalloc(&P->d_sponge, 12 * m));
  acc(dmalloc(&P->d_fa, 4 * n)); acc(dmalloc(&P->d_fcoef, 2 * m)); acc(dmalloc(&P->d_fcoef2, 2 * m));
  acc(dmalloc(&P->d_pow, 1));
  if (rc) { sbn_prover_destroy(P); return rc; }
  P->d_fb = P->d_fa + 2 * n;
  hipc(hipMalloc((void**)&P->d_pic, sizeof(ExpPiConsts<F>)), "hipMalloc");
  hipc(hipMalloc((void**)&P->d_idx, cfg->num_query_rounds * sizeof(u32)), "hipMalloc");
  {
    u32 bits = P->lde_log;
    for (u32 ab : P->fri.arity_bits) {
      u64* v = nullptr; acc(dmalloc(&v, 2 * ((size_t)1 << bits))); P->fri_vals.push_back(v);
      DevTree t; acc(tree_alloc(t, (size_t)1 << (bits - ab), cfg->cap_height)); P->fri_trees.push_back(t);
      bits -= ab;
    }
    if (rc) { sbn_prover_destroy(P); return rc; }
  }
  {
    size_t sib = (size_t)(P->lde_log - cfg->cap_height) * 4;
    size_t s = C + sib + (Z ? Z + sib : 0) + 4 + sib;
    u32 bits = P->lde_log;
    for (u32 ab : P->fri.arity_bits) { bits -= ab; s += 2 * ((size_t)1 << ab) + (size_t)(bits - cfg->cap_height) * 4; }
    P->qstride = s;
    acc(dmalloc(&P->d_qbuf, s * cfg->num_query_rounds));
    if (rc) { sbn_prover_destroy(P); return rc; }
  }
  auto blocks = [](size_t k) { return dim3((unsigned)((k + 255) / 256)); };
  F w = f_root_of_unity(P->lde_log);
  hipLaunchKernelGGL(pow_table_kernel, blocks(m), dim3(256), 0, P->stream, P->d_tw_f, m, w.v);
  hipLaunchKernelGGL(pow_table_kernel, blocks(m), dim3(256), 0, P->stream, P->d_tw_i, m, f_inv(w).v);
  hipLaunchKernelGGL(pow_table_kernel, blocks(m), dim3(256), 0, P->stream, P->d_shift, m, (u64)GL_GEN);
  hipLaunchKernelGGL(pow_table_kernel, blocks(m), dim3(256), 0, P->stream, P->d_shift_inv, m, f_inv(F(GL_GEN)).v);
  hipLaunchKernelGGL(domain_tables_kernel, blocks(m), dim3(256), 0, P->stream, P->d_xs, P->d_lag_first, P->d_lag_last, m, P->lde_log, degree_bits);
  if (P->d_shift_odd) hipLaunchKernelGGL(shift_odd_table_kernel, blocks(n), dim3(256), 0, P->stream, P->d_shift_odd, n, P->d_shift, P->d_tw_f, 9u);
  {
    std::vector<PairCols> pairs(Z);
    for (size_t z = 0; z < Z; z++) {
      int l, r;
      if (as.kind == SBN_AIR_G1_OP) G1OpShape::pair((int)z, l, r);
      else if (as.kind == SBN_AIR_LOOKUP) LookupShape().pair((int)z, l, r);
      else if (is_op_air(as.kind)) OpShape(as.kind).pair((int)z, l, r);
      else exp_shape(as).pair((int)z, l, r);
      pairs[z].lhs = l; pairs[z].rhs = r;
    }
    hipc(hipMalloc((void**)&P->d_pairs, std::max<size_t>(Z, 1) * sizeof(PairCols)), "hipMalloc");
    if (!rc && Z) hipc(hipMemcpy(P->d_pairs, pairs.data(), Z * sizeof(PairCols), hipMemcpyHostToDevice), "hipMemcpy");
    if (P->sp && P->sp->zr) {
      SplitCtx* S = P->sp;
      std::vector<PairCols> own(S->zr);
      for (size_t l = 0; l < S->zr; l++) own[l] = pairs[S->zs.global_col(S->zs.rank, l)];
      hipc(hipMalloc((void**)&S->d_pairs_own, S->zr * sizeof(PairCols)), "hipMalloc");
      if (!rc) hipc(hipMemcpy(S->d_pairs_own, own.data(), S->zr * sizeof(PairCols), hipMemcpyHostToDevice), "hipMemcpy");
    }
  }
  hipc(hipStreamSynchronize(P->stream), "hipStreamSynchronize");
  hipc(hipGetLastError(), "table kernels");
  if (rc) { sbn_prover_destroy(P); return rc; }
  *out = P;
  return SBN_OK;
}

extern "C" void sbn_prover_destroy(sbn_prover* P) {
  if (!P) return;
  (void)hipSetDevice(P->device);
  if (P->rc_pending) (void)hipEventSynchronize(P->rc_done);
  u64* bufs[] = {P->d_trace, P->d_coef, P->d_lde, P->d_tmp, P->d_tmp2, P->d_tmp3, P->d_zval, P->d_zcoef, P->d_zlde, P->d_q, P->d_qlde, P->tree_t.d, P->tree_z.d,
                 P->tree_q.d, P->d_tw_f, P->d_tw_i, P->d_shift, P->d_shift_inv, P->d_xs, P->d_lag_first, P->d_lag_last, P->d_apow, P->d_zpow,
                 P->d_open, P->d_part, P->d_w, P->d_fa, P->d_fcoef, P->d_fcoef2, P->d_pow, P->d_qbuf, P->d_shift_odd};
  for (u64* b : bufs) if (b) (void)hipFree(b);
  for (u64* b : P->fri_vals) if (b) (void)hipFree(b);
  for (auto& t : P->fri_trees) if (t.d) (void)hipFree(t.d);
  if (P->sp) {
    if (P->sp->d_ldechunk) (void)hipFree(P->sp->d_ldechunk);
    if (P->sp->d_idx_local) (void)hipFree(P->sp->d_idx_local);
    if (P->sp->d_pairs_own) (void)hipFree(P->sp->d_pairs_own);
    for (auto& e : P->sp->xchg_done) if (e) (void)hipEventDestroy(e);
    for (auto& e : P->sp->tev) if (e) (void)hipEventDestroy(e);
    if (P->sp->cstream) (void)hipStreamDestroy(P->sp->cstream);
    delete P->sp;
  }
  if (P->d_pic) (void)hipFree(P->d_pic);
  if (P->d_idx) (void)hipFree(P->d_idx);
  if (P->d_pairs) (void)hipFree(P->d_pairs);
  for (auto& e : P->ev) if (e) (void)hipEventDestroy(e);
  for (auto& e : P->abs_ev) if (e) (void)hipEventDestroy(e);
  for (auto& e : P->chunk_ready) if (e) (void)hipEventDestroy(e);
  if (P->hash_done) (void)hipEventDestroy(P->hash_done);
  if (P->d_sponge) (void)hipFree(P->d_sponge);
  if (P->h_chain) (void)hipHostFree(P->h_chain);
  if (P->h_io) (void)hipHostFree(P->h_io);
  if (P->h_open) (void)hipHostFree(P->h_open);
  if (P->h_open2) (void)hipHostFree(P->h_open2);
  if (P->hstream) (void)hipStreamDestroy(P->hstream);
  if (P->rstream) (void)hipStreamDestroy(P->rstream);
  if (P->rows_done) (void)hipEventDestroy(P->rows_done);
  if (P->rc_done) (void)hipEventDestroy(P->rc_done);
  if (P->d_rc_err) (void)hipFree(P->d_rc_err);
  if (P->nstream) { (void)hipStreamDestroy(P->nstream); for (auto& e : P->intt_done) if (e) (void)hipEventDestroy(e); }
  if (P->stream) (void)hipStreamDestroy(P->stream);
  delete P;
}

static int check_pi(sbn_prover* P, const uint64_t* pi, size_t n_pi) {
  if (n_pi != P->air.npi) return fail(SBN_ERR_BAD_ARG, "expected %zu public inputs, got %zu", P->air.npi, n_pi);
  if (n_pi && !pi) return fail(SBN_ERR_BAD_ARG, "null public inputs");
  for (size_t i = 0; i < n_pi; i++) if (pi[i] >= GLP) return fail(SBN_ERR_NON_CANONICAL, "public input %zu is not canonical", i);
  P->pi.assign(pi, pi + n_pi);
  return 0;
}
static int rc_finish(sbn_prover* P) {
  if (!P->rc_pending) return SBN_OK;
  P->rc_pending = false;
  int err = 0;
  HIPC(hipEventSynchronize(P->rc_done));
  HIPC(hipMemcpy(&err, P->d_rc_err, sizeof(int), hipMemcpyDeviceToHost));
  if (err) { P->loaded = false; return fail(SBN_ERR_WITNESS, "range-checked column holds a value >= 2^16"); }
  return SBN_OK;
}
extern "C" int sbn_prover_load_trace(sbn_prover* P, const uint64_t* trace, const uint64_t* pi, size_t n_pi) {
  if (!P || !trace) return fail(SBN_ERR_BAD_ARG, "null argument");
  int rc = check_pi(P, pi, n_pi); if (rc) return rc;
  (void)rc_finish(P);
  size_t words = P->air.ncols * P->n;
  {
    unsigned nt = std::thread::hardware_concurrency(); if (nt == 0) nt = 4; if (nt > 16) nt = 16;
    std::atomic<size_t> bad(words);
    std::vector<std::thread> th;
    size_t per = (words + nt - 1) / nt;
    for (unsigned t = 0; t < nt; t++)
      th.emplace_back([&, t] {
        size_t a = t * per, b = std::min(words, a + per);
        for (size_t i = a; i < b; i++) if (trace[i] >= GLP) { size_t cur = bad.load(); while (i < cur && !bad.compare_exchange_weak(cur, i)) {} break; }
      });
    for (auto& x : th) x.join();
    if (bad.load() < words) return fail(SBN_ERR_NON_CANONICAL, "trace word %zu is not canonical", bad.load());
  }
  HIPC(hipSetDevice(P->device));
  HIPC(hipMemcpy(P->d_trace, trace, words * sizeof(u64), hipMemcpyHostToDevice));
  P->loaded = true;
  return SBN_OK;
}
extern "C" int sbn_prover_load_trace_device(sbn_prover* P, const uint64_t* d_trace, const uint64_t* pi, size_t n_pi) {
  if (!P || !d_trace) return fail(SBN_ERR_BAD_ARG, "null argument");
  int rc = check_pi(P, pi, n_pi); if (rc) return rc;
  HIPC(hipSetDevice(P->device));
  (void)rc_finish(P);
  if (d_trace != P->d_trace) HIPC(hipMemcpy(P->d_trace, d_trace, P->air.ncols * P->n * sizeof(u64), hipMemcpyDeviceToDevice));
  P->loaded = true;
  return SBN_OK;
}
static int range_check_setup(int device) {
  static std::atomic<bool> done[SBN_MAX_DEVICES];
  const int d = device >= 0 && device < SBN_MAX_DEVICES ? device : 0;
  if (!done[d].load()) {
    HIPC(hipFuncSetAttribute((const void*)tg::range_check_kernel<false>, hipFuncAttributeMaxDynamicSharedMemorySize, (int)tg::RC_LDS_BYTES));
    HIPC(hipFuncSetAttribute((const void*)tg::range_check_kernel<true>, hipFuncAttributeMaxDynamicSharedMemorySize, (int)tg::RC_LDS_BYTES));
    done[d].store(true);
  }
  return 0;
}
struct ChainProgram {
  std::vector<uint32_t> ops[2];
  int levels[2] = {0, 0};
  int slots = 0;
};
static ChainProgram build_chain_program(int E) {
  struct Op { int kind, d, a, b, level; };
  struct Val { int s[2]; };
  ChainProgram out;
  for (int bit = 0; bit < 2; bit++) {
    std::vector<int> lvl;
    std::vector<Op> ops;
    auto fresh = [&](int level) { lvl.push_back(level); return (int)lvl.size() - 1; };
    auto emit = [&](int kind, int a, int b) { const int L = 1 + std::max(lvl[a], lvl[b]); const int d = fresh(L); ops.push_back({kind, d, a, b, L}); return d; };
    auto add = [&](Val x, Val y) { Val r{}; for (int q = 0; q < E; q++) r.s[q] = emit(tg::CP_ADD, x.s[q], y.s[q]); return r; };
    auto sub = [&](Val x, Val y) { Val r{}; for (int q = 0; q < E; q++) r.s[q] = emit(tg::CP_SUB, x.s[q], y.s[q]); return r; };
    auto mul = [&](Val x, Val y) {
      Val r{};
      if (E == 1) { r.s[0] = emit(tg::CP_MUL, x.s[0], y.s[0]); return r; }
      const int t0 = emit(tg::CP_MUL, x.s[0], y.s[0]), t1 = emit(tg::CP_MUL, x.s[1], y.s[1]);
      const int t2 = emit(tg::CP_MUL, x.s[0], y.s[1]), t3 = emit(tg::CP_MUL, x.s[1], y.s[0]);
      r.s[0] = emit(tg::CP_SUB, t0, t1); r.s[1] = emit(tg::CP_ADD, t2, t3);
      return r;
    };
    auto chk_zero = [&](Val x) {
      const int a = x.s[0], b = E == 2 ? x.s[1] : x.s[0];
      ops.push_back({E == 2 ? tg::CP_CHK2 : tg::CP_CHK1, 0, a, b, 1 + std::max(lvl[a], lvl[b])});
    };
    Val pa[3], pb[3];
    for (int c = 0; c < 3; c++) for (int q = 0; q < E; q++) pa[c].s[q] = fresh(0);
    for (int c = 0; c < 3; c++) for (int q = 0; q < E; q++) pb[c].s[q] = fresh(0);
    Val nb[3] = {pb[0], pb[1], pb[2]};
    if (bit) {
      const Val Z1Z1 = mul(pb[2], pb[2]), Z2Z2 = mul(pa[2], pa[2]);
      const Val U1 = mul(pb[0], Z2Z2), U2 = mul(pa[0], Z1Z1);
      const Val S1 = mul(mul(pb[1], pa[2]), Z2Z2), S2 = mul(mul(pa[1], pb[2]), Z1Z1);
      const Val H = sub(U2, U1);
      chk_zero(H);
      const Val H2 = add(H, H), I = mul(H2, H2), J = mul(H, I);
      const Val rr0 = sub(S2, S1), r = add(rr0, rr0);
      const Val V = mul(U1, I);
      nb[0] = sub(sub(mul(r, r), J), add(V, V));
      const Val sj = mul(S1, J);
      nb[1] = sub(mul(r, sub(V, nb[0])), add(sj, sj));
      const Val zs = add(pb[2], pa[2]);
      nb[2] = mul(sub(sub(mul(zs, zs), Z1Z1), Z2Z2), H);
    }
    chk_zero(pa[1]);
    Val na[3];
    {
      const Val A = mul(pa[0], pa[0]), B = mul(pa[1], pa[1]), C = mul(B, B);
      const Val t0 = add(pa[0], B), t1 = mul(t0, t0), t2 = sub(sub(t1, A), C);
      const Val D = add(t2, t2), Ee = add(add(A, A), A), F = mul(Ee, Ee);
      na[0] = sub(F, add(D, D));
      const Val C2 = add(C, C), C4 = add(C2, C2), C8 = add(C4, C4);
      na[1] = sub(mul(Ee, sub(D, na[0])), C8);
      const Val yz = mul(pa[1], pa[2]);
      na[2] = add(yz, yz);
    }
    int top = 0;
    for (const Op& o : ops) top = std::max(top, o.level);
    for (int c = 0; c < 3; c++) for (int q = 0; q < E; q++) {
      ops.push_back({tg::CP_COPY, pa[c].s[q], na[c].s[q], na[c].s[q], top + 1});
      if (bit) ops.push_back({tg::CP_COPY, pb[c].s[q], nb[c].s[q], nb[c].s[q], top + 1});
    }
    const int nl = top + 1;
    out.levels[bit] = nl;
    out.slots = std::max(out.slots, (int)lvl.size());
    out.ops[bit].assign((size_t)nl * tg::CP_LANES, 0u);
    std::vector<int> fill(nl, 0);
    for (const Op& o : ops) {
      const int L = o.level - 1;
      if (fill[L] >= tg::CP_LANES || (int)lvl.size() > tg::CP_MAX_SLOTS) { out.levels[0] = out.levels[1] = -1; return out; }
      out.ops[bit][(size_t)L * tg::CP_LANES + fill[L]++] = (uint32_t)o.kind | ((uint32_t)o.d << 8) | ((uint32_t)o.a << 16) | ((uint32_t)o.b << 24);
    }
  }
  return out;
}

template <int E>
static int generate_trace_device(sbn_prover* P, const uint32_t* ios, size_t K, uint64_t* pi_out) {
  const size_t n = P->n;
  const size_t IOW = 8 * (4 * E + 1);
  for (size_t k = 0; k < K; k++)
    for (int v = 0; v < 4 * E; v++) {
// ... 349 lines not shown
}

extern "C" int sbn_prover_prove(sbn_prover* P, sbn_proof** out) {
  if (!P || !out) return fail(SBN_ERR_BAD_ARG, "null argument");
  *out = nullptr;
  if (!P->loaded && !(P->sp && P->sp->comm.world > 1)) return fail(SBN_ERR_BAD_ARG, "no trace loaded");
  HIPC(hipSetDevice(P->device));
  hipStream_t st = P->stream;
  const size_t n = P->n, m = P->m, C = P->air.ncols, Z = P->air.nzs;
  const sbn_config& cfg = P->cfg;
  const size_t capw = ((size_t)1 << cfg.cap_height) * 4;
  auto blocks = [](size_t k) { return dim3((unsigned)((k + 255) / 256)); };
  int rc;
  Challenger ch;
  std::vector<u64> trace_cap, z_cap, q_cap;

  HIPC(hipEventRecord(P->ev[ST_TRACE_COMMIT], st));
  SplitCtx* const S = P->sp;
  struct DeadlineScope { ~DeadlineScope() { t_wait_deadline_s = 0; } } deadline_scope;
  if (S && S->comm.world > 1) {
    t_wait_deadline_s = P->set.comm_timeout_s;
    std::vector<uint32_t> st_all(S->comm.world, 0);
    const uint32_t mine = P->loaded ? 1u : 0u;
    if ((rc = split_all_gather_host(P, &mine, st_all.data(), sizeof(uint32_t)))) return rc;
    for (u32 r = 0; r < S->comm.world; r++) if (!st_all[r]) return fail(SBN_ERR_BAD_ARG, "split proof abandoned: rank %u has no trace loaded", r);
  }
  if (!P->loaded) return fail(SBN_ERR_BAD_ARG, "no trace loaded");
  if (S) {
    S->tev_used = 0;
    if (P->rc_pending) HIPC(hipStreamWaitEvent(st, P->rc_done, 0));
    if ((rc = commit_split(P, S->cs, P->d_trace, true, P->d_coef, S->lde_l, S->lde_n, P->tree_t))) return rc;
  } else if ((rc = commit_pipeline(P, P->d_trace, P->d_coef, P->d_lde, C, P->tree_t, EX_TRACE_ABSORB_MS, EX_TRACE_ABSORB_LAUNCHES))) return rc;
  HIPC(hipEventRecord(P->ev[ST_PERM_Z], st));
  if ((rc = S ? split_cap_to_host(P, P->tree_t, trace_cap) : tree_cap_to_host(P, P->tree_t, trace_cap))) return rc;
  if ((rc = rc_finish(P))) return rc;
  ch.observe_words(trace_cap.data(), capw);

  F gam[2][2] = {};
  if (Z) for (int s = 0; s < 2; s++) for (int c = 0; c < (int)cfg.num_challenges; c++) { (void)ch.challenge(); gam[s][c] = ch.challenge(); }
  const F gamma0 = gam[0][0], gamma1 = gam[1][1];
  {
    const size_t zn = S ? S->zr : Z;
    const PairCols* pairs = S ? S->d_pairs_own : P->d_pairs;
    auto launch_z = [&](size_t z0, size_t cnt, hipStream_t s) {
      if (cnt == 0) return;
      const PairCols* pp = pairs + z0; u64* out = P->d_zval + z0 * n;
      const size_t chunks = n / 2048;
      if (n >= 8192 && n % 2048 == 0 && P->set.perm_z != 1 && cnt <= 65535 && cnt * chunks * 4 <= 2 * 32 * n) {
        u64* tot = P->d_part; u64* pq = P->d_part + cnt * chunks * 2;
        hipLaunchKernelGGL(permz_chunk_products_kernel<8>, dim3((unsigned)chunks, (unsigned)cnt), dim3(256), 0, s, P->d_trace, n, pp, gamma0.v, gamma1.v, tot);
        hipLaunchKernelGGL(permz_chunk_scan_kernel, dim3((unsigned)cnt), dim3(64), 0, s, tot, (u32)chunks, pq);
        hipLaunchKernelGGL(permz_chunk_write_kernel<8>, dim3((unsigned)chunks, (unsigned)cnt), dim3(256), 0, s, P->d_trace, n, pp, gamma0.v, gamma1.v, pq, out);
        return;
      }
      if (n % 2048 == 0) hipLaunchKernelGGL(permutation_z_kernel<8>, dim3((unsigned)cnt), dim3(256), 0, s, P->d_trace, n, pp, gamma0.v, gamma1.v, out);
      else if (n % 1024 == 0) hipLaunchKernelGGL(permutation_z_kernel<4>, dim3((unsigned)cnt), dim3(256), 0, s, P->d_trace, n, pp, gamma0.v, gamma1.v, out);
      else hipLaunchKernelGGL(permutation_z_kernel<2>, dim3((unsigned)cnt), dim3(256), 0, s, P->d_trace, n, pp, gamma0.v, gamma1.v, out);
    };
    launch_z(0, zn, st);
  }
  HIPC(hipGetLastError());
  HIPC(hipEventRecord(P->ev[ST_Z_COMMIT], st));
  if (S) {
    if ((rc = commit_split(P, S->zs, P->d_zval, false, P->d_zcoef, S->zlde_l, S->zlde_n, P->tree_z))) return rc;
  } else {
    if (C > 4) if ((rc = absorb_times(P, C, EX_TRACE_ABSORB_MS))) return rc;
    if (Z) if ((rc = commit_pipeline(P, P->d_zval, P->d_zcoef, P->d_zlde, Z, P->tree_z, EX_Z_ABSORB_MS, EX_Z_ABSORB_LAUNCHES))) return rc;
  }
  HIPC(hipEventRecord(P->ev[ST_QUOTIENT_EVAL], st));
  if (Z) {
    if ((rc = S ? split_cap_to_host(P, P->tree_z, z_cap) : tree_cap_to_host(P, P->tree_z, z_cap))) return rc;
    ch.observe_words(z_cap.data(), capw);
  }

  F alphas[SBN_NCH];
  for (int j = 0; j < SBN_NCH; j++) alphas[j] = ch.challenge();
  {
    const size_t APN = P->apow_n;
    std::vector<u64> apow((size_t)SBN_NCH * APN);
    std::vector<F> ap[SBN_NCH];
    for (int j = 0; j < SBN_NCH; j++) {
      ap[j].resize(APN);
      F a(1);
      for (size_t k = 0; k < APN; k++) { ap[j][k] = a; apow[(size_t)j * APN + k] = a.v; a = a * alphas[j]; }
    }
    HIPC(hipMemcpyAsync(P->d_apow, apow.data(), apow.size() * sizeof(u64), hipMemcpyHostToDevice, st));
    if (is_exp_air(P->air.kind)) {
      static thread_local ExpPiConsts<F> pic;
      const F* app[SBN_NCH] = {ap[0].data(), ap[1].data()};
      std::vector<F> pif(P->pi.size());
      for (size_t i = 0; i < pif.size(); i++) pif[i] = F(P->pi[i]);
      exp_pi_consts<F>(exp_shape(P->air), app, pif.data(), pic);
      HIPC(hipMemcpyAsync(P->d_pic, &pic, sizeof(pic), hipMemcpyHostToDevice, st));
    }
    HIPC(stream_wait(st));
  }
  {
    QuotientParams qp{};
    qp.lde = P->d_lde; qp.zlde = P->d_zlde; qp.m = m; qp.next_step = 2;
    qp.lde_next = qp.lde; qp.zlde_next = qp.zlde; qp.row_shift = 0; qp.row_rho = 0;
    if (S) {
      qp.lde = S->lde_l; qp.zlde = S->zlde_l; qp.m = S->ml; qp.row_shift = S->log_r; qp.row_rho = S->rho;
      qp.lde_next = S->planes == 2 ? S->lde_n : S->lde_l; qp.zlde_next = S->planes == 2 ? S->zlde_n : S->zlde_l;
      qp.next_step = S->comm.world == 1 ? 2 : (S->comm.world == 2 ? 1 : 0);
    }
    qp.xs = P->d_xs; qp.lag_first = P->d_lag_first; qp.lag_last = P->d_lag_last;
    F gn = f_exp_pow2(F(GL_GEN), P->degree_bits);
    qp.zh_inv[0] = f_inv(gn - F(1)).v; qp.zh_inv[1] = f_inv(-gn - F(1)).v;
    qp.last = f_inv(f_root_of_unity(P->degree_bits)).v;
    for (int j = 0; j < SBN_NCH; j++) { qp.alpha[j] = alphas[j].v; qp.apow[j] = P->d_apow + (size_t)j * P->apow_n; }
    qp.gamma0 = gamma0.v; qp.gamma1 = gamma1.v; qp.num_zs = (int)Z; qp.num_io = (int)P->air.num_io; qp.pic = P->d_pic; qp.qout = P->d_q;
    if (S) qp.qout = (u64*)S->comm.send_buf;
    qp.part = P->d_part;
    {
      qp.zsplit = (int)(Z / 2);
      qp.lookups_in_perm = P->set.quotient_lookups == 1;
      const u64 n_tail = is_exp_air(P->air.kind) ? (u64)ExpShape(exp_e(P->air.kind), (int)P->air.num_io).num_tail_constraints() : 0;
      const u64 after[4] = {n_tail + 2 * (u64)Z, 2 * (u64)Z, 0, 0};
      qp.seg_count[0] = (int)(P->air.nconstraints - n_tail); qp.seg_count[1] = (int)n_tail;
      qp.seg_count[2] = qp.seg_count[3] = 2 * (int)Z;
      for (int sgm = 0; sgm < 4; sgm++) for (int j = 0; j < SBN_NCH; j++) qp.seg_shift[sgm][j] = f_pow(alphas[j], after[sgm]).v;
    }
    const size_t qblocks = (qp.m + 255) / 256;
    qp.seg_mask = 0xfu;
#ifdef SBN_DIAG
    { const char* e = std::getenv("SBN_DIAG_QUOTIENT_SEGMASK"); if (e) qp.seg_mask = (u32)atoi(e) & 0xfu; }
    if (qp.seg_mask != 0xfu) HIPC(hipMemsetAsync(qp.part, 0, (size_t)QSEG * SBN_NCH * qp.m * sizeof(u64), st));
#endif
    HIPC(hipEventRecord(P->chunk_ready[3], st));
    HIPC(hipStreamWaitEvent(P->hstream, P->chunk_ready[3], 0));
    if ((rc = launch_quotient_parts(P, qp, qblocks))) return rc;
    HIPC(hipEventRecord(P->hash_done, P->hstream));
    HIPC(hipStreamWaitEvent(st, P->hash_done, 0));
    hipLaunchKernelGGL(quotient_combine_kernel, blocks(qp.m), dim3(256), 0, st, qp);
    HIPC(hipGetLastError());
    if (S) {
      if ((rc = split_all_gather_device(P, 2 * S->ml))) return rc;
      hipLaunchKernelGGL(split_unpack_rows_kernel, blocks(m), dim3(256), 0, st, S->scratch, m, 2u, S->log_r, P->d_q);
      HIPC(hipGetLastError());
    } else if (Z > 4) { if ((rc = absorb_times(P, Z, EX_Z_ABSORB_MS))) return rc; }
  }
  HIPC(hipEventRecord(P->ev[ST_QUOTIENT_COMMIT], st));
  if ((rc = ntt_columns(P, P->d_q, m, P->d_q, m, P->d_tmp, m, 2, P->lde_log, true, m, nullptr, P->d_shift_inv, host_inv_pow2(P->lde_log)))) return rc;
  if ((rc = lde_coeffs(P, P->d_q, P->d_qlde, 4))) return rc;
  if ((rc = tree_from_matrix(P, P->tree_q, P->d_qlde, 4))) return rc;
  HIPC(hipEventRecord(P->ev[ST_OPENINGS], st));
  if ((rc = tree_cap_to_host(P, P->tree_q, q_cap))) return rc;
  ch.observe_words(q_cap.data(), capw);

  E2 zeta = ch.ext_challenge();
  F g = f_root_of_unity(P->degree_bits);
  if (e2_exp_pow2(zeta, P->degree_bits) == E2(F(1), F(0))) return fail(SBN_ERR_HIP, "opening point is in the subgroup");
  E2 zeta_next = zeta * g;
  hipLaunchKernelGGL(ext_pow_table_kernel, blocks(n), dim3(256), 0, st, P->d_zpow, P->d_zpow + n, n, zeta.a.v, zeta.b.v);
  hipLaunchKernelGGL(ext_pow_table_kernel, blocks(n), dim3(256), 0, st, P->d_zpow + 2 * n, P->d_zpow + 3 * n, n, zeta_next.a.v, zeta_next.b.v);
  const u64* open = P->h_open;
  const u64* open2 = P->h_open2;
  if (S && S->comm.world > 1) {
    const u64 *zp0 = P->d_zpow, *zp1 = P->d_zpow + n, *zp2 = P->d_zpow + 2 * n, *zp3 = P->d_zpow + 3 * n;
    auto open_k = n % 1024 == 0 ? openings_kernel<4> : openings_kernel<1>;
    if (S->cr) hipLaunchKernelGGL(open_k, dim3((unsigned)S->cr), dim3(256), 0, st, P->d_coef, n, zp0, zp1, zp2, zp3, P->d_open);
    if (S->zr) hipLaunchKernelGGL(open_k, dim3((unsigned)S->zr), dim3(256), 0, st, P->d_zcoef, n, zp0, zp1, zp2, zp3, P->d_open + C * 4);
    hipLaunchKernelGGL(open_k, dim3(4), dim3(256), 0, st, P->d_q, n, zp0, zp1, zp2, zp3, P->d_open + (C + Z) * 4);
    HIPC(hipGetLastError());
    HIPC(hipMemcpyAsync(P->h_open, P->d_open, (C + Z + 4) * 4 * sizeof(u64), hipMemcpyDeviceToHost, st));
    HIPC(hipEventRecord(P->ev[ST_FRI_COMBINE], st));
    HIPC(stream_wait(st));
    const u32 R = S->comm.world;
    const size_t cmax = S->cs.max_own(), zmax = S->zs.max_own(), per = (cmax + zmax) * 4;
    std::vector<u64> mine(per, 0), all((size_t)R * per);
    memcpy(mine.data(), P->h_open, S->cr * 4 * sizeof(u64));
    memcpy(mine.data() + cmax * 4, P->h_open + C * 4, S->zr * 4 * sizeof(u64));
    if ((rc = split_all_gather_host(P, mine.data(), all.data(), per * sizeof(u64)))) return rc;
    for (u32 r = 0; r < R; r++) {
      const u64* src = all.data() + (size_t)r * per;
      for (size_t l = 0, cnt = S->cs.own_cols(r); l < cnt; l++) memcpy(P->h_open + S->cs.global_col(r, l) * 4, src + l * 4, 4 * sizeof(u64));
      for (size_t l = 0, cnt = S->zs.own_cols(r); l < cnt; l++) memcpy(P->h_open + (C + S->zs.global_col(r, l)) * 4, src + (cmax + l) * 4, 4 * sizeof(u64));
    }
    open2 = open;
    for (size_t p = 0; p < C + Z + 4; p++) { ch.observe(F(open[4 * p])); ch.observe(F(open[4 * p + 1])); }
    for (size_t p = 0; p < C + Z; p++) { ch.observe(F(open[4 * p + 2])); ch.observe(F(open[4 * p + 3])); }
  } else {
    const bool u4 = n % 1024 == 0;
    auto open1_k = u4 ? openings1_kernel<4> : openings1_kernel<1>;
    const u64 *zp0 = P->d_zpow, *zp1 = P->d_zpow + n, *zp2 = P->d_zpow + 2 * n, *zp3 = P->d_zpow + 3 * n;
    size_t sl[5] = {0, C / 16, C / 16 + C / 8, C / 16 + C / 8 + C / 4, C};
    for (int k = 0; k < 4; k++) {
      const size_t a = sl[k], cnt = sl[k + 1] - sl[k];
      if (cnt) {
        hipLaunchKernelGGL(open1_k, dim3((unsigned)cnt), dim3(256), 0, st, P->d_coef + a * n, n, zp0, zp1, P->d_open + a * 4, 0u);
        HIPC(hipMemcpyAsync(P->h_open + a * 4, P->d_open + a * 4, cnt * 4 * sizeof(u64), hipMemcpyDeviceToHost, st));
      }
      HIPC(hipEventRecord(P->chunk_ready[8 + k], st));
    }
    if (Z) hipLaunchKernelGGL(open1_k, dim3((unsigned)Z), dim3(256), 0, st, P->d_zcoef, n, zp0, zp1, P->d_open + C * 4, 0u);
    hipLaunchKernelGGL(open1_k, dim3(4), dim3(256), 0, st, P->d_q, n, zp0, zp1, P->d_open + (C + Z) * 4, 0u);
    HIPC(hipMemcpyAsync(P->h_open + C * 4, P->d_open + C * 4, (Z + 4) * 4 * sizeof(u64), hipMemcpyDeviceToHost, st));
    HIPC(hipEventRecord(P->chunk_ready[1], st));
    size_t sn[5] = {0, C / 4, C / 2, C / 2 + C / 4, C};
    for (int k = 0; k < 4; k++) {
      const size_t a = sn[k], cnt = sn[k + 1] - sn[k];
      if (cnt) {
        hipLaunchKernelGGL(open1_k, dim3((unsigned)cnt), dim3(256), 0, st, P->d_coef + a * n, n, zp2, zp3, P->d_open + a * 4, 2u);
        HIPC(hipMemcpyAsync(P->h_open2 + a * 4, P->d_open + a * 4, cnt * 4 * sizeof(u64), hipMemcpyDeviceToHost, st));
      }
      HIPC(hipEventRecord(P->chunk_ready[12 + k], st));
    }
    if (Z) hipLaunchKernelGGL(open1_k, dim3((unsigned)Z), dim3(256), 0, st, P->d_zcoef, n, zp2, zp3, P->d_open + C * 4, 2u);
    HIPC(hipGetLastError());
    HIPC(hipMemcpyAsync(P->h_open2 + C * 4, P->d_open + C * 4, Z * 4 * sizeof(u64), hipMemcpyDeviceToHost, st));
    HIPC(hipEventRecord(P->ev[ST_FRI_COMBINE], st));
    for (int k = 0; k < 4; k++) {
      HIPC(event_wait(P->chunk_ready[8 + k]));
      for (size_t p = sl[k]; p < sl[k + 1]; p++) { ch.observe(F(open[4 * p])); ch.observe(F(open[4 * p + 1])); }
    }
    HIPC(event_wait(P->chunk_ready[1]));
    for (size_t p = C; p < C + Z + 4; p++) { ch.observe(F(open[4 * p])); ch.observe(F(open[4 * p + 1])); }
    for (int k = 0; k < 4; k++) {
      HIPC(event_wait(P->chunk_ready[12 + k]));
      for (size_t p = sn[k]; p < sn[k + 1]; p++) { ch.observe(F(open2[4 * p + 2])); ch.observe(F(open2[4 * p + 3])); }
    }
    HIPC(stream_wait(st));
    for (size_t p = C; p < C + Z; p++) { ch.observe(F(open2[4 * p + 2])); ch.observe(F(open2[4 * p + 3])); }
  }

  E2 fri_alpha = ch.ext_challenge();
  {
    const u32 RW = S ? S->comm.world : 1;
    const u32 GS = RW > 1 ? (u32)SPLIT_BLOCK : 128;
    std::vector<u64> wall;
    auto plan = [&](u32 npoly, E2 weight0, u64 stride) { size_t off = wall.size(); u32 ng = (npoly + GS - 1) / GS; E2 ag = e2_pow(fri_alpha, stride), cur = weight0;
                                                         for (u32 k = 0; k < ng; k++) { wall.push_back(cur.a.v); wall.push_back(cur.b.v); cur = cur * ag; } return off; };
    const size_t tc0 = S ? (size_t)S->comm.rank * GS : 0, tcn = S ? S->cr : C, tzn = S ? S->zr : Z;
    const u64 gstride = (u64)GS * RW;
    size_t w_t = tcn ? plan((u32)tcn, e2_pow(fri_alpha, RW > 1 ? tc0 : 0), gstride) : 0, w_z = tzn ? plan((u32)tzn, e2_pow(fri_alpha, C + (RW > 1 ? tc0 : 0)), gstride) : 0,
           w_q = plan(4, e2_pow(fri_alpha, C + Z), GS);
    if (wall.size() > 4096) return fail(SBN_ERR_UNSUPPORTED, "too many FRI combine groups");
    HIPC(hipMemcpyAsync(P->d_w, wall.data(), wall.size() * sizeof(u64), hipMemcpyHostToDevice, st));
    hipLaunchKernelGGL(ext_pow_table_kernel, dim3(1), dim3(GS), 0, st, P->d_apow, P->d_apow + GS, (size_t)GS, fri_alpha.a.v, fri_alpha.b.v);
    auto combine = [&](const u64* coeffs, u32 npoly, size_t woff, u64* oa, u64* ob, int accumulate) -> int {
      u32 ng = (npoly + GS - 1) / GS;
      for (u32 g0 = 0; g0 < ng; g0 += 32) {
        u32 gc = std::min<u32>(32, ng - g0);
        hipLaunchKernelGGL(fri_combine_partial_kernel, dim3((unsigned)((n + 255) / 256), gc), dim3(256), 0, st, coeffs + (size_t)g0 * GS * n, n,
                           npoly - g0 * GS, GS, P->d_apow, P->d_apow + GS, P->d_part, P->d_part + 32 * n);
        hipLaunchKernelGGL(fri_combine_reduce_kernel, blocks(n), dim3(256), 0, st, P->d_part, P->d_part + 32 * n, n, gc, P->d_w + woff + 2 * g0, oa, ob,
                           (accumulate || g0 > 0) ? 1 : 0);
      }
      HIPC(hipGetLastError());
      return 0;
    };
    u64 *f1a = P->d_fb, *f1b = P->d_fb + n, *f0a = P->d_fa, *f0b = P->d_fa + n;
    if (!tcn) HIPC(hipMemsetAsync(f1a, 0, 2 * n * sizeof(u64), st));
    if (tcn) if ((rc = combine(P->d_coef, (u32)tcn, w_t, f1a, f1b, 0))) return rc;
    if (tzn) if ((rc = combine(P->d_zcoef, (u32)tzn, w_z, f1a, f1b, 1))) return rc;
    if (S) {
      HIPC(hipMemcpyAsync(S->comm.send_buf, f1a, 2 * n * sizeof(u64), hipMemcpyDeviceToDevice, st));
      if ((rc = split_all_gather_device(P, 2 * n))) return rc;
      hipLaunchKernelGGL(split_modadd_kernel, blocks(2 * n), dim3(256), 0, st, S->scratch, 2 * n, S->comm.world, f1a);
      HIPC(hipGetLastError());
    }
    HIPC(hipMemcpyAsync(f0a, f1a, 2 * n * sizeof(u64), hipMemcpyDeviceToDevice, st));
    if ((rc = combine(P->d_q, 4, w_q, f0a, f0b, 1))) return rc;
    HIPC(stream_wait(st));
    HIPC(hipMemsetAsync(P->d_fcoef, 0, 2 * m * sizeof(u64), st));
    E2 shift2 = e2_pow(fri_alpha, C + Z);
    auto divide = [&](const u64* ca, const u64* cb, E2 z, E2 mul, int accumulate) {
      const size_t nch = n / DBL_CHUNK;
      u64 *ha = P->d_part, *hb = P->d_part + nch;
      hipLaunchKernelGGL(divide_by_linear_pass1, blocks(nch), dim3(256), 0, st, ca, cb, nch, z.a.v, z.b.v, ha, hb);
      hipLaunchKernelGGL(divide_by_linear_pass2, dim3(1), dim3(256), 0, st, ha, hb, nch, z.a.v, z.b.v);
      hipLaunchKernelGGL(divide_by_linear_pass3, blocks(nch), dim3(256), 0, st, ca, cb, nch, z.a.v, z.b.v, ha, hb, mul.a.v, mul.b.v, P->d_fcoef, P->d_fcoef + m, accumulate, fri_times_x(cfg));
    };
    divide(f0a, f0b, zeta, E2{F(0), F(0)}, 0);
    divide(f1a, f1b, zeta_next, shift2, 1);
    HIPC(hipGetLastError());
  }
  HIPC(hipEventRecord(P->ev[ST_FRI_LAYERS], st));
  std::vector<std::vector<u64>> fri_caps;
  std::vector<u64> final_poly;
  {
    u32 bits = P->lde_log;
    u64* coef = P->d_fcoef; u64* coef_alt = P->d_fcoef2;
    size_t clen = m;
    F shift(GL_GEN);
    for (size_t li = 0; li < P->fri.arity_bits.size(); li++) {
      u32 ab = P->fri.arity_bits[li];
      u64* va = P->fri_vals[li]; u64* vb = va + clen;
      HIPC(hipMemcpyAsync(va, coef, 2 * clen * sizeof(u64), hipMemcpyDeviceToDevice, st));
      hipLaunchKernelGGL(scale_pow_kernel, blocks(clen), dim3(256), 0, st, va, clen, shift.v);
      hipLaunchKernelGGL(scale_pow_kernel, blocks(clen), dim3(256), 0, st, vb, clen, shift.v);
      if ((rc = ntt_columns(P, va, clen, va, clen, P->d_tmp, m, 2, bits, false, clen, nullptr, nullptr, 1))) return rc;
      DevTree& t = P->fri_trees[li];
      if (t.nleaf <= 16384) hipLaunchKernelGGL(fri_leaf_hash_coop_kernel, blocks(t.nleaf * 16), dim3(256), 0, st, va, vb, bits, ab, t.d);
      else hipLaunchKernelGGL(fri_leaf_hash_kernel, blocks(t.nleaf), dim3(256), 0, st, va, vb, bits, ab, t.d);
      if ((rc = tree_build_inner(P, t, st))) return rc;
      std::vector<u64> cap;
      if ((rc = tree_cap_to_host(P, t, cap))) return rc;
      ch.observe_words(cap.data(), capw);
      fri_caps.push_back(cap);
      E2 beta = ch.ext_challenge();
      size_t nout = clen >> ab;
      hipLaunchKernelGGL(fri_fold_kernel, blocks(nout), dim3(256), 0, st, coef, coef + clen, nout, 1u << ab, beta.a.v, beta.b.v, coef_alt, coef_alt + nout);
      HIPC(hipGetLastError());
      std::swap(coef, coef_alt);
      clen = nout; bits -= ab;
      shift = f_pow(shift, (u64)1 << ab);
    }
    size_t fl = clen >> cfg.rate_bits;
    final_poly.resize(2 * fl);
    std::vector<u64> fa(fl), fb(fl);
    HIPC(hipMemcpyAsync(fa.data(), coef, fl * sizeof(u64), hipMemcpyDeviceToHost, st));
    HIPC(hipMemcpyAsync(fb.data(), coef + clen, fl * sizeof(u64), hipMemcpyDeviceToHost, st));
    HIPC(stream_wait(st));
    for (size_t i = 0; i < fl; i++) { final_poly[2 * i] = fa[i]; final_poly[2 * i + 1] = fb[i]; ch.observe(F(fa[i])); ch.observe(F(fb[i])); }
  }
  HIPC(hipEventRecord(P->ev[ST_POW], st));
  u64 pow_witness = ~0ULL;
  {
    PowParams pp{};
    for (int i = 0; i < 12; i++) pp.state[i] = ch.st[i].v;
    for (size_t i = 0; i < ch.in.size(); i++) pp.state[i] = ch.in[i].v;
    pp.wpos = (u32)ch.in.size(); pp.min_lz = cfg.proof_of_work_bits; pp.result = P->d_pow;
    u64 base = 0;
    for (int round = 0; pow_witness == ~0ULL; round++) {
      const u64 BATCH = round == 0 ? (1ULL << 17) : (1ULL << 20);
      if (base >= GLP - BATCH) return fail(SBN_ERR_HIP, "proof of work failed");
      u64 init = ~0ULL;
      HIPC(hipMemcpyAsync(P->d_pow, &init, sizeof(u64), hipMemcpyHostToDevice, st));
      pp.base = base; pp.count = BATCH;
      hipLaunchKernelGGL(pow_kernel, blocks(BATCH), dim3(256), 0, st, pp);
      HIPC(hipMemcpyAsync(&pow_witness, P->d_pow, sizeof(u64), hipMemcpyDeviceToHost, st));
      HIPC(stream_wait(st));
      base += BATCH;
    }
    ch.observe(F(pow_witness));
    F resp = ch.challenge();
    u32 lz = resp.v ? (u32)__builtin_clzll(resp.v) : 64;
    if (lz < cfg.proof_of_work_bits) return fail(SBN_ERR_HIP, "proof-of-work witness check failed");
  }
  HIPC(hipEventRecord(P->ev[ST_QUERIES], st));
  const u32 nq = cfg.num_query_rounds;
  std::vector<u64> qwords(P->qstride * nq);
  std::vector<u32> idx(nq), idx_local(nq);
  size_t split_section = 0;
  {
    for (u32 q = 0; q < nq; q++) idx[q] = (u32)(ch.challenge().v % m);
    HIPC(hipMemcpyAsync(P->d_idx, idx.data(), nq * sizeof(u32), hipMemcpyHostToDevice, st));
    size_t off = 0;
    const u32 nsib = P->lde_log - cfg.cap_height;
    auto initial = [&](const u64* mat, size_t ncols, const DevTree& t, size_t rows, u32 log_rows, const u32* d_index) {
      hipLaunchKernelGGL(gather_rows_kernel, dim3((unsigned)((ncols + 255) / 256), nq), dim3(256), 0, st, mat, rows, log_rows, (u32)ncols, d_index, P->d_qbuf, P->qstride, off);
      off += ncols;
      hipLaunchKernelGGL(gather_siblings_kernel, dim3(nq), dim3(128), 0, st, t.d, t.nleaf, nsib, d_index, 0u, P->d_qbuf, P->qstride, off);
      off += (size_t)nsib * 4;
    };
    if (S) {
      for (u32 q = 0; q < nq; q++) idx_local[q] = idx[q] & (u32)(S->ml - 1);
      HIPC(hipMemcpyAsync(S->d_idx_local, idx_local.data(), nq * sizeof(u32), hipMemcpyHostToDevice, st));
      initial(S->lde_l, C, P->tree_t, S->ml, P->lde_log - S->log_r, S->d_idx_local);
      if (Z) initial(S->zlde_l, Z, P->tree_z, S->ml, P->lde_log - S->log_r, S->d_idx_local);
      split_section = off;
    } else {
      initial(P->d_lde, C, P->tree_t, m, P->lde_log, P->d_idx);
      if (Z) initial(P->d_zlde, Z, P->tree_z, m, P->lde_log, P->d_idx);
    }
    initial(P->d_qlde, 4, P->tree_q, m, P->lde_log, P->d_idx);
    u32 bits = P->lde_log, shift = 0;
    for (size_t li = 0; li < P->fri.arity_bits.size(); li++) {
      u32 ab = P->fri.arity_bits[li];
      shift += ab;
      size_t len = (size_t)1 << bits;
      hipLaunchKernelGGL(gather_fri_leaf_kernel, dim3(nq), dim3(64), 0, st, P->fri_vals[li], P->fri_vals[li] + len, bits, ab, P->d_idx, shift, P->d_qbuf, P->qstride, off);
      off += 2 * ((size_t)1 << ab);
      const DevTree& t = P->fri_trees[li];
      hipLaunchKernelGGL(gather_siblings_kernel, dim3(nq), dim3(128), 0, st, t.d, t.nleaf, t.nlevels, P->d_idx, shift, P->d_qbuf, P->qstride, off);
      off += (size_t)t.nlevels * 4;
      bits -= ab;
    }
    HIPC(hipGetLastError());
    if (off != P->qstride) return fail(SBN_ERR_HIP, "internal: query layout mismatch (%zu vs %zu)", off, P->qstride);
    HIPC(hipMemcpyAsync(qwords.data(), P->d_qbuf, qwords.size() * sizeof(u64), hipMemcpyDeviceToHost, st));
  }
  HIPC(hipEventRecord(P->ev[ST_COUNT], st));
  HIPC(stream_wait(st));
  for (int i = 0; i < ST_COUNT; i++) HIPC(hipEventElapsedTime(&P->stage_ms[i], P->ev[i], P->ev[i + 1]));
  if (S) {
    const u32 R = S->comm.world;
    std::vector<u64> mine((size_t)nq * split_section), all((size_t)R * nq * split_section);
    for (u32 q = 0; q < nq; q++) memcpy(mine.data() + (size_t)q * split_section, qwords.data() + (size_t)q * P->qstride, split_section * sizeof(u64));
    if ((rc = split_all_gather_host(P, mine.data(), all.data(), mine.size() * sizeof(u64)))) return rc;
    for (u32 q = 0; q < nq; q++) {
      const u32 owner = idx[q] >> (P->lde_log - S->log_r);
      memcpy(qwords.data() + (size_t)q * P->qstride, all.data() + ((size_t)owner * nq + q) * split_section, split_section * sizeof(u64));
    }
    float xms = 0;
    for (size_t i = 0; i + 1 < S->tev_used; i += 2) { float t = 0; HIPC(hipEventElapsedTime(&t, S->tev[i], S->tev[i + 1])); xms += t; }
    P->stage_ms[ST_COUNT + EX_COMM_MS] = xms;
  }

  sbn_proof* pr = new sbn_proof();
  pr->degree_bits = P->degree_bits;
  std::vector<u64>& w = pr->words;
  w.reserve(12 + 3 * capw + (C + Z + 4) * 4 + fri_caps.size() * capw + qwords.size() + final_poly.size() + 1 + P->pi.size());
  u64 hdr[12] = {PROOF_MAGIC, P->degree_bits, C, Z, 4, P->pi.size(), cfg.cap_height, cfg.rate_bits, fri_caps.size(), cfg.fri_arity_bits,
                 final_poly.size() / 2, nq};
  w.insert(w.end(), hdr, hdr + 12);
  w.insert(w.end(), trace_cap.begin(), trace_cap.end());
  if (Z) w.insert(w.end(), z_cap.begin(), z_cap.end());
  w.insert(w.end(), q_cap.begin(), q_cap.end());
  for (size_t p = 0; p < C; p++) { w.push_back(open[4 * p]); w.push_back(open[4 * p + 1]); }
  for (size_t p = 0; p < C; p++) { w.push_back(open2[4 * p + 2]); w.push_back(open2[4 * p + 3]); }
  for (size_t p = C; p < C + Z; p++) { w.push_back(open[4 * p]); w.push_back(open[4 * p + 1]); }
  for (size_t p = C; p < C + Z; p++) { w.push_back(open2[4 * p + 2]); w.push_back(open2[4 * p + 3]); }
  for (size_t p = C + Z; p < C + Z + 4; p++) { w.push_back(open[4 * p]); w.push_back(open[4 * p + 1]); }
  for (auto& cap : fri_caps) w.insert(w.end(), cap.begin(), cap.end());
  w.insert(w.end(), qwords.begin(), qwords.end());
  w.insert(w.end(), final_poly.begin(), final_poly.end());
  w.push_back(pow_witness);
  w.insert(w.end(), P->pi.begin(), P->pi.end());
  *out = pr;
  return SBN_OK;
}

extern "C" int sbn_commit_values(const uint64_t* cols, size_t ncols, size_t n, uint32_t rate_bits, uint32_t cap_height, uint64_t* cap_out,
                                 uint64_t* coeffs_out, uint64_t* lde_out) {
  if (!cols || !cap_out || ncols == 0) return fail(SBN_ERR_BAD_ARG, "null argument");
  if (rate_bits != 1 || n < 512 || (n & (n - 1))) return fail(SBN_ERR_UNSUPPORTED, "need rate_bits=1 and n a power of two >= 512");
  u32 lg = 0; while (((size_t)1 << lg) < n) lg++;
  sbn_prover P{};
  sbn_standard_fast_config(&P.cfg); P.cfg.cap_height = cap_height;
  P.degree_bits = lg; P.lde_log = lg + 1; P.n = n; P.m = 2 * n; P.ntt_chunk = 64; P.device = g_device;
  int ndev = 0;
  if (hipGetDeviceCount(&ndev) != hipSuccess || ndev == 0) return fail(SBN_ERR_NO_DEVICE, "no HIP device available: no CPU fallback");
  HIPC(hipSetDevice(g_device));
  { int rc0 = ntt_fast_setup(); if (rc0) return rc0; }
  { std::string serr; if (!P.set.load(serr)) return fail(SBN_ERR_BAD_ARG, "%s", serr.c_str()); }
  P.fast_ntt = P.set.fast_ntt; P.ntt_xcd = P.set.ntt_xcd;
  P.ntt_fused = P.fast_ntt && (lg == 16 || lg == 17) && P.set.ntt_fused;
  P.ntt_fused512 = P.fast_ntt && lg == 18 && P.set.ntt_split1024 && P.set.ntt_fused;
  HIPC(hipStreamCreate(&P.stream));
  u64 *d_vals = nullptr, *d_coef = nullptr, *d_lde = nullptr;
  int rc = 0;
  rc |= dmalloc(&d_vals, ncols * n); rc |= dmalloc(&d_coef, ncols * n); rc |= dmalloc(&d_lde, ncols * P.m); rc |= dmalloc(&P.d_tmp, 64 * P.m);
  if (P.ntt_fused || P.ntt_fused512) rc |= dmalloc(&P.d_tmp2, 64 * P.m);
  if (lg == 18 && P.set.ntt_split1024) rc |= dmalloc(&P.d_shift_odd, n);
  rc |= dmalloc(&P.d_tw_f, P.m); rc |= dmalloc(&P.d_tw_i, P.m); rc |= dmalloc(&P.d_shift, P.m);
  rc |= tree_alloc(P.tree_t, P.m, cap_height);
  if (!rc) {
    auto blocks = [](size_t k) { return dim3((unsigned)((k + 255) / 256)); };
    F w = f_root_of_unity(P.lde_log);
    hipLaunchKernelGGL(pow_table_kernel, blocks(P.m), dim3(256), 0, P.stream, P.d_tw_f, P.m, w.v);
    hipLaunchKernelGGL(pow_table_kernel, blocks(P.m), dim3(256), 0, P.stream, P.d_tw_i, P.m, f_inv(w).v);
    hipLaunchKernelGGL(pow_table_kernel, blocks(P.m), dim3(256), 0, P.stream, P.d_shift, P.m, (u64)GL_GEN);
    if (P.d_shift_odd) hipLaunchKernelGGL(shift_odd_table_kernel, blocks(n), dim3(256), 0, P.stream, P.d_shift_odd, n, P.d_shift, P.d_tw_f, 9u);
    if (hipMemcpy(d_vals, cols, ncols * n * sizeof(u64), hipMemcpyHostToDevice) != hipSuccess) rc = fail(SBN_ERR_HIP, "H2D failed");
  }
  for (size_t c0 = 0; !rc && c0 < ncols; c0 += P.ntt_chunk) rc = intt_then_lde_chunk(&P, d_vals, d_coef, d_lde, c0, std::min(P.ntt_chunk, ncols - c0));
  if (!rc && ncols <= 4) rc = tree_from_matrix(&P, P.tree_t, d_lde, ncols);
  if (!rc && ncols > 4) {
    rc = dmalloc(&P.d_sponge, 12 * P.m);
    for (size_t c0 = 0; !rc && c0 < ncols; c0 += 64) {
      size_t nc = std::min<size_t>(64, ncols - c0);
      hipLaunchKernelGGL(leaf_absorb_kernel, dim3((unsigned)((P.m + 255) / 256)), dim3(256), 0, P.stream, d_lde + c0 * P.m, P.m, P.lde_log, (u32)nc, P.d_sponge,
                         c0 == 0 ? 1 : 0, c0 + 64 >= ncols ? 1 : 0, P.tree_t.d, (c0 + 64 < ncols && ncols - (c0 + 64) >= 8) ? 1 : 0);
    }
    if (!rc) rc = tree_build_inner(&P, P.tree_t, P.stream);
  }
  std::vector<u64> cap;
  if (!rc) rc = tree_cap_to_host(&P, P.tree_t, cap);
  if (!rc) memcpy(cap_out, cap.data(), cap.size() * sizeof(u64));
  if (!rc && coeffs_out && hipMemcpy(coeffs_out, d_coef, ncols * n * sizeof(u64), hipMemcpyDeviceToHost) != hipSuccess) rc = fail(SBN_ERR_HIP, "D2H failed");
  if (!rc && lde_out && hipMemcpy(lde_out, d_lde, ncols * P.m * sizeof(u64), hipMemcpyDeviceToHost) != hipSuccess) rc = fail(SBN_ERR_HIP, "D2H failed");
  for (u64* b : {d_vals, d_coef, d_lde, P.d_tmp, P.d_tmp2, P.d_shift_odd, P.d_tw_f, P.d_tw_i, P.d_shift, P.tree_t.d, P.d_sponge}) if (b) (void)hipFree(b);
  (void)hipStreamDestroy(P.stream);
  return rc;
}

extern "C" int sbn_poseidon_permute_batch(uint64_t* states, size_t count) {
  if (!states) return fail(SBN_ERR_BAD_ARG, "null argument");
  int ndev = 0;
  if (hipGetDeviceCount(&ndev) != hipSuccess || ndev == 0) return fail(SBN_ERR_NO_DEVICE, "no HIP device available: no CPU fallback");
  HIPC(hipSetDevice(g_device));
  for (size_t i = 0; i < count * 12; i++) if (states[i] >= GLP) return fail(SBN_ERR_NON_CANONICAL, "state word %zu is not canonical", i);
  u64* d = nullptr;
  HIPC(hipMalloc((void**)&d, count * 12 * sizeof(u64)));
  HIPC(hipMemcpy(d, states, count * 12 * sizeof(u64), hipMemcpyHostToDevice));
  hipLaunchKernelGGL(poseidon_batch_kernel, dim3((unsigned)((count + 255) / 256)), dim3(256), 0, 0, d, count);
  HIPC(hipMemcpy(states, d, count * 12 * sizeof(u64), hipMemcpyDeviceToHost));
  (void)hipFree(d);
  return SBN_OK;
}

extern "C" int sbn_field_mul_batch(const uint64_t* a, const uint64_t* b, uint64_t* out, size_t count, int mode) {
  if (!a || !b || !out) return fail(SBN_ERR_BAD_ARG, "null argument");
  int ndev = 0;
  if (hipGetDeviceCount(&ndev) != hipSuccess || ndev == 0) return fail(SBN_ERR_NO_DEVICE, "no HIP device available: no CPU fallback");
  HIPC(hipSetDevice(g_device));
  if (count == 0) return SBN_OK;
  u64* d = nullptr;
  HIPC(hipMalloc((void**)&d, 3 * count * sizeof(u64)));
  hipError_t e = hipMemcpy(d, a, count * sizeof(u64), hipMemcpyHostToDevice);
  if (e == hipSuccess) e = hipMemcpy(d + count, b, count * sizeof(u64), hipMemcpyHostToDevice);
  if (e == hipSuccess) {
    hipLaunchKernelGGL(field_mul_batch_kernel, dim3((unsigned)((count + 255) / 256)), dim3(256), 0, 0, d, d + count, d + 2 * count, count, mode);
    e = hipMemcpy(out, d + 2 * count, count * sizeof(u64), hipMemcpyDeviceToHost);
  }
  (void)hipFree(d);
  if (e != hipSuccess) return fail(SBN_ERR_HIP, "sbn_field_mul_batch: %s", hipGetErrorString(e));
  return SBN_OK;
}

extern "C" int sbn_bn254_fq_batch(int op, const uint64_t* a, const uint64_t* b, uint64_t* out, size_t count, int on_device) {
  using namespace tg;
  if (op < FQB_MUL || op > FQB_FQ2_INV) return fail(SBN_ERR_BAD_ARG, "unknown op %d", op);
  const bool binary = op == FQB_MUL || op == FQB_ADD || op == FQB_SUB || op == FQB_FQ2_INV;
  if (!a || !out || (binary && !b)) return fail(SBN_ERR_BAD_ARG, "null argument");
  if (op == FQB_BATCH_INV && count % TG_INV_BATCH) return fail(SBN_ERR_BAD_ARG, "batch inverse needs a multiple of %d values", TG_INV_BATCH);
  for (size_t i = 0; i < count; i++) {
    if (bnw::geq_p(a + 4 * i) || (binary && bnw::geq_p(b + 4 * i))) return fail(SBN_ERR_NON_CANONICAL, "element %zu is not below p", i);
    const bool za = !(a[4 * i] | a[4 * i + 1] | a[4 * i + 2] | a[4 * i + 3]);
    const bool zb = !binary || !(b[4 * i] | b[4 * i + 1] | b[4 * i + 2] | b[4 * i + 3]);
    if ((op == FQB_INV || op == FQB_BATCH_INV) && za) return fail(SBN_ERR_BAD_ARG, "element %zu is zero: no inverse", i);
    if (op == FQB_FQ2_INV && za && zb) return fail(SBN_ERR_BAD_ARG, "element %zu is zero: no inverse", i);
  }
  const size_t items = op == FQB_BATCH_INV ? count / TG_INV_BATCH : count, out_words = 4 * count * (op == FQB_FQ2_INV ? 2 : 1);
  if (!on_device) {
    for (size_t i = 0; i < items; i++) fq_batch_item(op, a, b, out, i);
    return SBN_OK;
  }
  int ndev = 0;
  if (hipGetDeviceCount(&ndev) != hipSuccess || ndev == 0) return fail(SBN_ERR_NO_DEVICE, "no HIP device available: no CPU fallback");
  HIPC(hipSetDevice(g_device));
  if (count == 0) return SBN_OK;
  u64* d = nullptr;
  HIPC(hipMalloc((void**)&d, (8 * count + out_words) * sizeof(u64)));
  hipError_t e = hipMemcpy(d, a, 4 * count * sizeof(u64), hipMemcpyHostToDevice);
  if (e == hipSuccess && binary) e = hipMemcpy(d + 4 * count, b, 4 * count * sizeof(u64), hipMemcpyHostToDevice);
  if (e == hipSuccess) {
    hipLaunchKernelGGL(fq_batch_kernel, dim3((unsigned)((items + 63) / 64)), dim3(64), 0, 0, op, d, d + 4 * count, d + 8 * count, items);
    e = hipGetLastError();
    if (e == hipSuccess) e = hipMemcpy(out, d + 8 * count, out_words * sizeof(u64), hipMemcpyDeviceToHost);
  }
  (void)hipFree(d);
  if (e != hipSuccess) return fail(SBN_ERR_HIP, "sbn_bn254_fq_batch: %s", hipGetErrorString(e));
  return SBN_OK;
}

extern "C" int sbn_poseidon_permute_host(uint64_t* states, size_t count, int use_definition) {
  if (!states) return fail(SBN_ERR_BAD_ARG, "null argument");
  for (size_t i = 0; i < count * 12; i++) if (states[i] >= GLP) return fail(SBN_ERR_NON_CANONICAL, "state word %zu is not canonical", i);
  for (size_t k = 0; k < count; k++) {
    F st[12];
    for (int i = 0; i < 12; i++) st[i] = F(states[12 * k + i]);
    if (use_definition) poseidon_permute_generic(st); else poseidon_permute(st);
    for (int i = 0; i < 12; i++) states[12 * k + i] = st[i].v;
  }
  return SBN_OK;
}

extern "C" int sbn_set_device(int device) {
  int ndev = 0;
  if (hipGetDeviceCount(&ndev) != hipSuccess || device < 0 || device >= ndev) return fail(SBN_ERR_NO_DEVICE, "device %d not available", device);
  HIPC(hipSetDevice(device));
  t_device = device; g_default_device.store(device);
  return SBN_OK;
}
// ... 64 lines not shown
```

Before: 44.52.

## Fuse opening passes, precompute FRI shift tables, use pinned transfers, speed host Poseidon

Result: no change. 44.21, median of 2 (-0.7%).

```diff
diff --git a/starky_bn254_amd/csrc/kernels.cuh b/starky_bn254_amd/csrc/kernels.cuh
--- a/starky_bn254_amd/csrc/kernels.cuh
+++ b/starky_bn254_amd/csrc/kernels.cuh
@@ -11,10 +11,6 @@
 __global__ void shift_odd_table_kernel(u64* out, size_t n, const u64* __restrict__ shift, const u64* __restrict__ tw, u32 log_s) {
   size_t i = (size_t)blockIdx.x * blockDim.x + threadIdx.x;
   if (i < n) out[i] = (F(shift[i]) * F(tw[(i >> log_s) << log_s])).v;
-}
-__global__ void scale_pow_kernel(u64* v, size_t n, u64 base) {
-  size_t i = (size_t)blockIdx.x * blockDim.x + threadIdx.x;
-  if (i < n) v[i] = (F(v[i]) * f_pow(F(base), i)).v;
 }
 
 __global__ __launch_bounds__(256) __attribute__((amdgpu_waves_per_eu(4))) void leaf_hash_kernel(const u64* __restrict__ lde, size_t m, u32 lde_log, u32 ncols,
@@ -523,6 +519,12 @@
   E2 r = e2_pow(E2(F(z0), F(z1)), i);
   pa[i] = r.a.v; pb[i] = r.b.v;
 }
+__global__ void ext_pow_table2_kernel(u64* p, size_t n, u64 z0, u64 z1, u64 w0, u64 w1) {
+  size_t i = (size_t)blockIdx.x * blockDim.x + threadIdx.x;
+  if (i >= n) return;
+  const E2 r = e2_pow(E2(F(z0), F(z1)), i), t = e2_pow(E2(F(w0), F(w1)), i);
+  p[i] = r.a.v; p[n + i] = r.b.v; p[2 * n + i] = t.a.v; p[3 * n + i] = t.b.v;
+}
 __device__ __forceinline__ F block_sum(F v, u64* sh) {
   const int lane = threadIdx.x & 63, wv = threadIdx.x >> 6;
 #pragma unroll
@@ -534,19 +536,19 @@
   for (unsigned w = 0; w < blockDim.x / 64; w++) t = t + F(sh[w]);
   return t;
 }
-template <u32 OPEN_UNROLL>
-__global__ __launch_bounds__(256) void openings_kernel(const u64* __restrict__ coeffs, size_t n, const u64* __restrict__ pa0, const u64* __restrict__ pb0,
-                                                       const u64* __restrict__ pa1, const u64* __restrict__ pb1, u64* __restrict__ out) {
-  __shared__ u64 sh[4];
+template <u32 OPEN_UNROLL, u32 NT = 256>
+__global__ __launch_bounds__(NT) void openings_kernel(const u64* __restrict__ coeffs, size_t n, const u64* __restrict__ pa0, const u64* __restrict__ pb0,
+                                                      const u64* __restrict__ pa1, const u64* __restrict__ pb1, u64* __restrict__ out) {
+  __shared__ u64 sh[NT / 64];
   const u64* c = coeffs + (size_t)blockIdx.x * n;
   Acc<F> s0, r0, s1, r1;
   s0.clear(); r0.clear(); s1.clear(); r1.clear();
-  for (size_t i = threadIdx.x; i < n; i += 256 * OPEN_UNROLL) {
+  for (size_t i = threadIdx.x; i < n; i += NT * OPEN_UNROLL) {
     u64 cv[OPEN_UNROLL], t0[OPEN_UNROLL], t1[OPEN_UNROLL], t2[OPEN_UNROLL], t3[OPEN_UNROLL];
 #pragma unroll
     for (u32 k = 0; k < OPEN_UNROLL; k++) {
-      const size_t ik = i + 256 * k;
-      cv[k] = c[ik]; t0[k] = pa0[ik]; t1[k] = pb0[ik]; t2[k] = pa1[ik]; t3[k] = pb1[ik];
+      const size_t ik = i + NT * k;
+      cv[k] = __builtin_nontemporal_load(c + ik); t0[k] = pa0[ik]; t1[k] = pb0[ik]; t2[k] = pa1[ik]; t3[k] = pb1[ik];
     }
     __builtin_amdgcn_sched_barrier(0);
 #pragma unroll
@@ -560,34 +562,6 @@
   if (threadIdx.x == 0) {
     u64* o = out + (size_t)blockIdx.x * 4;
     o[0] = a0.v; o[1] = b0.v; o[2] = a1.v; o[3] = b1.v;
-  }
-}
-
-template <u32 OPEN_UNROLL>
-__global__ __launch_bounds__(256) void openings1_kernel(const u64* __restrict__ coeffs, size_t n, const u64* __restrict__ pa, const u64* __restrict__ pb,
-                                                        u64* __restrict__ out, u32 off) {
-  __shared__ u64 sh[4];
-  const u64* c = coeffs + (size_t)blockIdx.x * n;
-  Acc<F> s0, r0;
-  s0.clear(); r0.clear();
-  for (size_t i = threadIdx.x; i < n; i += 256 * OPEN_UNROLL) {
-    u64 cv[OPEN_UNROLL], t0[OPEN_UNROLL], t1[OPEN_UNROLL];
-#pragma unroll
-    for (u32 k = 0; k < OPEN_UNROLL; k++) {
-      const size_t ik = i + 256 * k;
-      cv[k] = c[ik]; t0[k] = pa[ik]; t1[k] = pb[ik];
-    }
-    __builtin_amdgcn_sched_barrier(0);
-#pragma unroll
-    for (u32 k = 0; k < OPEN_UNROLL; k++) {
-      const F v{cv[k]};
-      s0.macv(v, F(t0[k])); r0.macv(v, F(t1[k]));
-    }
-  }
-  const F a0 = block_sum(s0.value(), sh), b0 = block_sum(r0.value(), sh);
-  if (threadIdx.x == 0) {
-    u64* o = out + (size_t)blockIdx.x * 4 + off;
-    o[0] = a0.v; o[1] = b0.v;
   }
 }
 
diff --git a/starky_bn254_amd/csrc/poseidon.cuh b/starky_bn254_amd/csrc/poseidon.cuh
--- a/starky_bn254_amd/csrc/poseidon.cuh
+++ b/starky_bn254_amd/csrc/poseidon.cuh
@@ -402,29 +402,33 @@
   const __m512i y2 = mulred_x8(y, y), y4 = mulred_x8(y2, y2), y3 = mulred_x8(y2, y);
   return mulred_x8(y4, y3);
 }
-PH_AVX512 static void full_round_sboxes_avx512(u64* s, const u64* rc) {
-  const __m512i a = sbox7_x8(_mm512_loadu_si512(s), _mm512_loadu_si512(rc));
-  const __m512i b = sbox7_x8(_mm512_maskz_loadu_epi64(0x0F, s + 8), _mm512_maskz_loadu_epi64(0x0F, rc + 8));
-  _mm512_storeu_si512(s, a);
-  _mm512_mask_storeu_epi64(s + 8, 0x0F, b);
+struct MdsVecs { alignas(64) u64 a[12][8]; alignas(64) u64 b[12][8]; };
+static constexpr MdsVecs mds_vecs() {
+  constexpr u64 C[12] = {17, 15, 41, 16, 2, 28, 13, 13, 39, 18, 34, 20};
+  MdsVecs v{};
+  for (int j = 0; j < 12; j++)
+    for (int r = 0; r < 8; r++) {
+      v.a[j][r] = C[(j - r + 12) % 12] + (j == 0 && r == 0 ? 8 : 0);
+      v.b[j][r] = r < 4 ? C[(j - r - 8 + 24) % 12] : 0;
+    }
+  return v;
+}
+alignas(64) static constexpr MdsVecs MDS_V = mds_vecs();
+PH_AVX512 static inline __m512i tree12(const __m512i* t) {
+  const __m512i a = _mm512_add_epi64(_mm512_add_epi64(t[0], t[1]), _mm512_add_epi64(t[2], t[3]));
+  const __m512i b = _mm512_add_epi64(_mm512_add_epi64(t[4], t[5]), _mm512_add_epi64(t[6], t[7]));
+  const __m512i c = _mm512_add_epi64(_mm512_add_epi64(t[8], t[9]), _mm512_add_epi64(t[10], t[11]));
+  return _mm512_add_epi64(_mm512_add_epi64(a, b), c);
 }
 PH_AVX512 static inline void mds_x12(__m512i& A, __m512i& B) {
-  static const u64 C[12] = {17, 15, 41, 16, 2, 28, 13, 13, 39, 18, 34, 20};
   const __m512i M32 = _mm512_set1_epi64(0xFFFFFFFFLL);
-  const __m512i lane = _mm512_set_epi64(7, 6, 5, 4, 3, 2, 1, 0);
-  const __m512i twelve = _mm512_set1_epi64(12);
-  __m512i slA = _mm512_setzero_si512(), shA = slA, slB = slA, shB = slA;
+  __m512i la[12], ha[12], lb[12], hb[12];
 #pragma GCC unroll 12
-  for (int i = 0; i < 12; i++) {
-    __m512i ia = _mm512_add_epi64(lane, _mm512_set1_epi64(i));
-    ia = _mm512_mask_sub_epi64(ia, _mm512_cmpge_epu64_mask(ia, twelve), ia, twelve);
-    __m512i ib = _mm512_add_epi64(lane, _mm512_set1_epi64((i + 8) % 12));
-    ib = _mm512_mask_sub_epi64(ib, _mm512_cmpge_epu64_mask(ib, twelve), ib, twelve);
-    const __m512i xa = _mm512_permutex2var_epi64(A, ia, B), xb = _mm512_permutex2var_epi64(A, ib, B);
-    const __m512i ca = i == 0 ? _mm512_set_epi64(17, 17, 17, 17, 17, 17, 17, 25) : _mm512_set1_epi64((long long)C[i]);
-    const __m512i cb = _mm512_set1_epi64((long long)C[i]);
-    slA = _mm512_add_epi64(slA, _mm512_mul_epu32(xa, ca)); shA = _mm512_add_epi64(shA, _mm512_mul_epu32(_mm512_srli_epi64(xa, 32), ca));
-    slB = _mm512_add_epi64(slB, _mm512_mul_epu32(xb, cb)); shB = _mm512_add_epi64(shB, _mm512_mul_epu32(_mm512_srli_epi64(xb, 32), cb));
+  for (int j = 0; j < 12; j++) {
+    const __m512i x = _mm512_permutexvar_epi64(_mm512_set1_epi64(j & 7), j < 8 ? A : B), xh = _mm512_srli_epi64(x, 32);
+    const __m512i ca = _mm512_load_si512(MDS_V.a[j]), cb = _mm512_load_si512(MDS_V.b[j]);
+    la[j] = _mm512_mul_epu32(x, ca); ha[j] = _mm512_mul_epu32(xh, ca);
+    lb[j] = _mm512_mul_epu32(x, cb); hb[j] = _mm512_mul_epu32(xh, cb);
   }
   auto fold = [&](__m512i sl, __m512i sh) PH_AVX512 {
     const __m512i shl = _mm512_slli_epi64(sh, 32);
@@ -436,10 +440,9 @@
     const __m512i r = _mm512_add_epi64(l, t1);
     return _mm512_mask_add_epi64(r, _mm512_cmplt_epu64_mask(r, t1), r, M32);
   };
-  A = fold(slA, shA); B = fold(slB, shB);
-}
-PH_AVX512 static void full_rounds_x4_avx512(u64* s, const u64* rc) {
-  __m512i A = _mm512_loadu_si512(s), B = _mm512_maskz_loadu_epi64(0x0F, s + 8);
+  A = fold(tree12(la), tree12(ha)); B = fold(tree12(lb), tree12(hb));
+}
+PH_AVX512 static inline void full_rounds_x4_avx512(__m512i& A, __m512i& B, const u64* rc) {
   for (int k = 0; k < 4; k++) {
     A = sbox7_x8(A, _mm512_loadu_si512(rc + 12 * k));
     B = sbox7_x8(B, _mm512_maskz_loadu_epi64(0x0F, rc + 12 * k + 8));
@@ -448,8 +451,14 @@
   const __m512i P = _mm512_set1_epi64((long long)GLP);
   A = _mm512_mask_sub_epi64(A, _mm512_cmpge_epu64_mask(A, P), A, P);
   B = _mm512_mask_sub_epi64(B, _mm512_cmpge_epu64_mask(B, P), B, P);
-  _mm512_storeu_si512(s, A);
-  _mm512_mask_storeu_epi64(s + 8, 0x0F, B);
+}
+PH_AVX512 static inline void full_rounds_x4_avx512(u64* s, const u64* rc) {
+  __m512i A = _mm512_set_epi64(s[7], s[6], s[5], s[4], s[3], s[2], s[1], s[0]);
+  __m512i B = _mm512_set_epi64(0, 0, 0, 0, s[11], s[10], s[9], s[8]);
+  full_rounds_x4_avx512(A, B, rc);
+  alignas(64) u64 o[16];
+  _mm512_store_si512(o, A); _mm512_store_si512(o + 8, B);
+  for (int i = 0; i < 12; i++) s[i] = o[i];
 }
 static inline bool host_has_avx512() {
   static const bool have = __builtin_cpu_supports("avx512f") && __builtin_cpu_supports("avx512dq") && !sbn::Settings::from_env_or_default().no_avx512;
@@ -482,7 +491,38 @@
   }();
   return T;
 }
+namespace ph {
+static inline u64 mulw(u64 a, u64 b) {
+  const u128 p = (u128)a * b;
+  const u64 lo = (u64)p, hi = (u64)(p >> 64), hi_hi = hi >> 32, hi_lo = hi & GLEPS;
+  u64 t0 = lo - hi_hi;
+  if (lo < hi_hi) t0 -= GLEPS;
+  const u64 t1 = (hi_lo << 32) - hi_lo;
+  u64 r = t0 + t1;
+  if (r < t1) r += GLEPS;
+  return r;
+}
+static inline u64 sbox7w(u64 x) { const u64 x2 = mulw(x, x), x4 = mulw(x2, x2), x3 = mulw(x2, x); return mulw(x4, x3); }
+static inline u64 fold_weak(const Acc& a) {
+  const u128 t = a.lo + a.hi * (u128)GLEPS;
+  const u64 lo = (u64)t, hi = (u64)(t >> 64), hi_hi = hi >> 32, hi_lo = hi & GLEPS;
+  u64 t0 = lo - hi_hi;
+  if (lo < hi_hi) t0 -= GLEPS;
+  const u64 t1 = (hi_lo << 32) - hi_lo;
+  u64 r = t0 + t1;
+  if (r < t1) r += GLEPS;
+  return r;
+}
+static inline u64 add_small_mul(u64 base, u64 t, u64 m) {
+  const u128 p = (u128)t * m + base;
+  const u64 lo = (u64)p, h = (u64)(p >> 64) * GLEPS;
+  u64 r = lo + h;
+  if (r < h) r += GLEPS;
+  return r;
+}
+}
 static inline void poseidon_permute_host_fast(F* s) {
+  static_assert(PFAST_M00 < (1ULL << 32), "the chain's multiply-add assumes a small M00");
   const u64* rc = POSEIDON_EFF_HOST;
   int r = 0;
   full_rounds_host(s, rc, r);
@@ -493,13 +533,18 @@
   ph::Acc fin[11];
   for (int i = 0; i < 11; i++) for (int j = 0; j < 11; j++) ph::mac(fin[i], PFAST_INIT[11 * i + j], u[j]);
   ph::Acc nxt; for (int j = 0; j < 11; j++) ph::mac(nxt, T.PI[0][j], u[j]);
-  u64 cur = s[0].v;
+  u64 in = s[0].v, cur = 0;
   for (int k = 0; k < 22; k++, r++) {
-    t[k] = sbox7(k ? F(cur) + F(rc[12 * r]) : F(cur)).v;
+    t[k] = ph::sbox7w(in);
     ph::Acc a = nxt;
     for (int q = 0; q < k; q++) ph::mac(a, T.K[k][q], t[q]);
-    ph::mac(a, PFAST_M00, t[k]);
-    cur = ph::fold(a);
+    if (k + 1 < 22) {
+      a.lo += rc[12 * (r + 1)];
+      in = ph::add_small_mul(ph::fold_weak(a), t[k], PFAST_M00);
+    } else {
+      ph::mac(a, PFAST_M00, t[k]);
+      cur = ph::fold(a);
+    }
     nxt = ph::Acc();
     if (k + 1 < 22) for (int j = 0; j < 11; j++) ph::mac(nxt, T.PI[k + 1][j], u[j]);
     for (int i = 0; i < 11; i++) ph::mac(fin[i], PFAST_WHAT[11 * k + i], t[k]);
diff --git a/starky_bn254_amd/csrc/prover.hip b/starky_bn254_amd/csrc/prover.hip
--- a/starky_bn254_amd/csrc/prover.hip
+++ b/starky_bn254_amd/csrc/prover.hip
@@ -97,6 +97,7 @@
   u64 *d_fcoef = nullptr;
   u64 *d_fcoef2 = nullptr;
   std::vector<u64*> fri_vals;
+  std::vector<u64*> fri_shift;
   u64 *d_pow = nullptr;
   u32 *d_idx = nullptr;
   u64 *d_qbuf = nullptr; size_t qstride = 0;
@@ -133,7 +134,9 @@
   u64* h_io = nullptr;
   size_t h_io_words = 0;
   u64* h_open = nullptr;
-  u64* h_open2 = nullptr;
+  u64* h_w = nullptr;
+  u64* h_xfer = nullptr;
+  size_t h_xfer_words = 0;
 };
 
 static int dmalloc(u64** p, size_t words) {
@@ -513,8 +516,10 @@
 static int tree_cap_to_host(sbn_prover* P, const DevTree& t, std::vector<u64>& cap) {
   size_t capn = (size_t)1 << P->cfg.cap_height;
   cap.resize(capn * 4);
-  HIPC(hipMemcpyAsync(cap.data(), t.level(t.nlevels), capn * 4 * sizeof(u64), hipMemcpyDeviceToHost, P->stream));
+  u64* dst = P->h_xfer ? P->h_xfer : cap.data();
+  HIPC(hipMemcpyAsync(dst, t.level(t.nlevels), capn * 4 * sizeof(u64), hipMemcpyDeviceToHost, P->stream));
   HIPC(stream_wait(P->stream));
+  if (dst != cap.data()) memcpy(cap.data(), dst, capn * 4 * sizeof(u64));
   return 0;
 }
 
@@ -658,7 +663,7 @@
   acc(dmalloc(&P->d_apow, (size_t)SBN_NCH * P->apow_n));
   acc(dmalloc(&P->d_zpow, 4 * n)); acc(dmalloc(&P->d_open, (C + Z + 4) * 4));
   hipc(hipHostMalloc((void**)&P->h_open, (C + Z + 4) * 4 * sizeof(u64), hipHostMallocDefault), "hipHostMalloc");
-  hipc(hipHostMalloc((void**)&P->h_open2, (C + Z) * 4 * sizeof(u64), hipHostMallocDefault), "hipHostMalloc");
+  hipc(hipHostMalloc((void**)&P->h_w, 4096 * sizeof(u64), hipHostMallocDefault), "hipHostMalloc");
   acc(dmalloc(&P->d_part, 2 * 32 * n)); acc(dmalloc(&P->d_w, 4096)); acc(dmalloc(&P->d_sponge, 12 * m));
   acc(dmalloc(&P->d_fa, 4 * n)); acc(dmalloc(&P->d_fcoef, 2 * m)); acc(dmalloc(&P->d_fcoef2, 2 * m));
   acc(dmalloc(&P->d_pow, 1));
@@ -670,9 +675,13 @@
     u32 bits = P->lde_log;
     for (u32 ab : P->fri.arity_bits) {
       u64* v = nullptr; acc(dmalloc(&v, 2 * ((size_t)1 << bits))); P->fri_vals.push_back(v);
+      u64* sh = nullptr; if (bits != P->lde_log) acc(dmalloc(&sh, (size_t)1 << bits)); P->fri_shift.push_back(sh);
       DevTree t; acc(tree_alloc(t, (size_t)1 << (bits - ab), cfg->cap_height)); P->fri_trees.push_back(t);
       bits -= ab;
     }
+    if (rc) { sbn_prover_destroy(P); return rc; }
+    P->h_xfer_words = std::max<size_t>((size_t)4 << cfg->cap_height, (size_t)2 << bits);
+    hipc(hipHostMalloc((void**)&P->h_xfer, P->h_xfer_words * sizeof(u64), hipHostMallocDefault), "hipHostMalloc");
     if (rc) { sbn_prover_destroy(P); return rc; }
   }
   {
@@ -693,6 +702,16 @@
   hipLaunchKernelGGL(domain_tables_kernel, blocks(m), dim3(256), 0, P->stream, P->d_xs, P->d_lag_first, P->d_lag_last, m, P->lde_log, degree_bits);
   if (P->d_shift_odd) hipLaunchKernelGGL(shift_odd_table_kernel, blocks(n), dim3(256), 0, P->stream, P->d_shift_odd, n, P->d_shift, P->d_tw_f, 9u);
   {
+    u32 bits = P->lde_log;
+    F shift(GL_GEN);
+    for (size_t li = 0; li < P->fri.arity_bits.size(); li++) {
+      if (li == 0) P->fri_shift[0] = P->d_shift;
+      else hipLaunchKernelGGL(pow_table_kernel, blocks((size_t)1 << bits), dim3(256), 0, P->stream, P->fri_shift[li], (size_t)1 << bits, shift.v);
+      shift = f_pow(shift, (u64)1 << P->fri.arity_bits[li]);
+      bits -= P->fri.arity_bits[li];
+    }
+  }
+  {
     std::vector<PairCols> pairs(Z);
     for (size_t z = 0; z < Z; z++) {
       int l, r;
@@ -728,6 +747,7 @@
                  P->d_open, P->d_part, P->d_w, P->d_fa, P->d_fcoef, P->d_fcoef2, P->d_pow, P->d_qbuf, P->d_shift_odd};
   for (u64* b : bufs) if (b) (void)hipFree(b);
   for (u64* b : P->fri_vals) if (b) (void)hipFree(b);
+  for (size_t li = 1; li < P->fri_shift.size(); li++) if (P->fri_shift[li]) (void)hipFree(P->fri_shift[li]);
   for (auto& t : P->fri_trees) if (t.d) (void)hipFree(t.d);
   if (P->sp) {
     if (P->sp->d_ldechunk) (void)hipFree(P->sp->d_ldechunk);
@@ -749,7 +769,8 @@
   if (P->h_chain) (void)hipHostFree(P->h_chain);
   if (P->h_io) (void)hipHostFree(P->h_io);
   if (P->h_open) (void)hipHostFree(P->h_open);
-  if (P->h_open2) (void)hipHostFree(P->h_open2);
+  if (P->h_w) (void)hipHostFree(P->h_w);
+  if (P->h_xfer) (void)hipHostFree(P->h_xfer);
   if (P->hstream) (void)hipStreamDestroy(P->hstream);
   if (P->rstream) (void)hipStreamDestroy(P->rstream);
   if (P->rows_done) (void)hipEventDestroy(P->rows_done);
@@ -1405,13 +1426,11 @@
   F g = f_root_of_unity(P->degree_bits);
   if (e2_exp_pow2(zeta, P->degree_bits) == E2(F(1), F(0))) return fail(SBN_ERR_HIP, "opening point is in the subgroup");
   E2 zeta_next = zeta * g;
-  hipLaunchKernelGGL(ext_pow_table_kernel, blocks(n), dim3(256), 0, st, P->d_zpow, P->d_zpow + n, n, zeta.a.v, zeta.b.v);
-  hipLaunchKernelGGL(ext_pow_table_kernel, blocks(n), dim3(256), 0, st, P->d_zpow + 2 * n, P->d_zpow + 3 * n, n, zeta_next.a.v, zeta_next.b.v);
+  hipLaunchKernelGGL(ext_pow_table2_kernel, blocks(n), dim3(256), 0, st, P->d_zpow, n, zeta.a.v, zeta.b.v, zeta_next.a.v, zeta_next.b.v);
   const u64* open = P->h_open;
-  const u64* open2 = P->h_open2;
+  const u64 *zp0 = P->d_zpow, *zp1 = P->d_zpow + n, *zp2 = P->d_zpow + 2 * n, *zp3 = P->d_zpow + 3 * n;
+  auto open_k = n % 1024 == 0 ? openings_kernel<4> : openings_kernel<1>;
   if (S && S->comm.world > 1) {
-    const u64 *zp0 = P->d_zpow, *zp1 = P->d_zpow + n, *zp2 = P->d_zpow + 2 * n, *zp3 = P->d_zpow + 3 * n;
-    auto open_k = n % 1024 == 0 ? openings_kernel<4> : openings_kernel<1>;
     if (S->cr) hipLaunchKernelGGL(open_k, dim3((unsigned)S->cr), dim3(256), 0, st, P->d_coef, n, zp0, zp1, zp2, zp3, P->d_open);
     if (S->zr) hipLaunchKernelGGL(open_k, dim3((unsigned)S->zr), dim3(256), 0, st, P->d_zcoef, n, zp0, zp1, zp2, zp3, P->d_open + C * 4);
     hipLaunchKernelGGL(open_k, dim3(4), dim3(256), 0, st, P->d_q, n, zp0, zp1, zp2, zp3, P->d_open + (C + Z) * 4);
@@ -1430,66 +1449,51 @@
       for (size_t l = 0, cnt = S->cs.own_cols(r); l < cnt; l++) memcpy(P->h_open + S->cs.global_col(r, l) * 4, src + l * 4, 4 * sizeof(u64));
       for (size_t l = 0, cnt = S->zs.own_cols(r); l < cnt; l++) memcpy(P->h_open + (C + S->zs.global_col(r, l)) * 4, src + (cmax + l) * 4, 4 * sizeof(u64));
     }
-    open2 = open;
     for (size_t p = 0; p < C + Z + 4; p++) { ch.observe(F(open[4 * p])); ch.observe(F(open[4 * p + 1])); }
     for (size_t p = 0; p < C + Z; p++) { ch.observe(F(open[4 * p + 2])); ch.observe(F(open[4 * p + 3])); }
   } else {
-    const bool u4 = n % 1024 == 0;
-    auto open1_k = u4 ? openings1_kernel<4> : openings1_kernel<1>;
-    const u64 *zp0 = P->d_zpow, *zp1 = P->d_zpow + n, *zp2 = P->d_zpow + 2 * n, *zp3 = P->d_zpow + 3 * n;
     size_t sl[5] = {0, C / 16, C / 16 + C / 8, C / 16 + C / 8 + C / 4, C};
+    const bool wide = n % 4096 == 0;
+    auto one_k = wide ? openings_kernel<4, 1024> : open_k;
+    const dim3 nt(wide ? 1024 : 256);
     for (int k = 0; k < 4; k++) {
       const size_t a = sl[k], cnt = sl[k + 1] - sl[k];
       if (cnt) {
-        hipLaunchKernelGGL(open1_k, dim3((unsigned)cnt), dim3(256), 0, st, P->d_coef + a * n, n, zp0, zp1, P->d_open + a * 4, 0u);
+        hipLaunchKernelGGL(one_k, dim3((unsigned)cnt), nt, 0, st, P->d_coef + a * n, n, zp0, zp1, zp2, zp3, P->d_open + a * 4);
         HIPC(hipMemcpyAsync(P->h_open + a * 4, P->d_open + a * 4, cnt * 4 * sizeof(u64), hipMemcpyDeviceToHost, st));
       }
       HIPC(hipEventRecord(P->chunk_ready[8 + k], st));
     }
-    if (Z) hipLaunchKernelGGL(open1_k, dim3((unsigned)Z), dim3(256), 0, st, P->d_zcoef, n, zp0, zp1, P->d_open + C * 4, 0u);
-    hipLaunchKernelGGL(open1_k, dim3(4), dim3(256), 0, st, P->d_q, n, zp0, zp1, P->d_open + (C + Z) * 4, 0u);
+    if (Z) hipLaunchKernelGGL(one_k, dim3((unsigned)Z), nt, 0, st, P->d_zcoef, n, zp0, zp1, zp2, zp3, P->d_open + C * 4);
+    hipLaunchKernelGGL(one_k, dim3(4), nt, 0, st, P->d_q, n, zp0, zp1, zp2, zp3, P->d_open + (C + Z) * 4);
+    HIPC(hipGetLastError());
     HIPC(hipMemcpyAsync(P->h_open + C * 4, P->d_open + C * 4, (Z + 4) * 4 * sizeof(u64), hipMemcpyDeviceToHost, st));
-    HIPC(hipEventRecord(P->chunk_ready[1], st));
-    size_t sn[5] = {0, C / 4, C / 2, C / 2 + C / 4, C};
-    for (int k = 0; k < 4; k++) {
-      const size_t a = sn[k], cnt = sn[k + 1] - sn[k];
-      if (cnt) {
-        hipLaunchKernelGGL(open1_k, dim3((unsigned)cnt), dim3(256), 0, st, P->d_coef + a * n, n, zp2, zp3, P->d_open + a * 4, 2u);
-        HIPC(hipMemcpyAsync(P->h_open2 + a * 4, P->d_open + a * 4, cnt * 4 * sizeof(u64), hipMemcpyDeviceToHost, st));
-      }
-      HIPC(hipEventRecord(P->chunk_ready[12 + k], st));
-    }
-    if (Z) hipLaunchKernelGGL(open1_k, dim3((unsigned)Z), dim3(256), 0, st, P->d_zcoef, n, zp2, zp3, P->d_open + C * 4, 2u);
-    HIPC(hipGetLastError());
-    HIPC(hipMemcpyAsync(P->h_open2 + C * 4, P->d_open + C * 4, Z * 4 * sizeof(u64), hipMemcpyDeviceToHost, st));
     HIPC(hipEventRecord(P->ev[ST_FRI_COMBINE], st));
     for (int k = 0; k < 4; k++) {
       HIPC(event_wait(P->chunk_ready[8 + k]));
       for (size_t p = sl[k]; p < sl[k + 1]; p++) { ch.observe(F(open[4 * p])); ch.observe(F(open[4 * p + 1])); }
     }
-    HIPC(event_wait(P->chunk_ready[1]));
+    HIPC(stream_wait(st));
     for (size_t p = C; p < C + Z + 4; p++) { ch.observe(F(open[4 * p])); ch.observe(F(open[4 * p + 1])); }
-    for (int k = 0; k < 4; k++) {
-      HIPC(event_wait(P->chunk_ready[12 + k]));
-      for (size_t p = sn[k]; p < sn[k + 1]; p++) { ch.observe(F(open2[4 * p + 2])); ch.observe(F(open2[4 * p + 3])); }
-    }
-    HIPC(stream_wait(st));
-    for (size_t p = C; p < C + Z; p++) { ch.observe(F(open2[4 * p + 2])); ch.observe(F(open2[4 * p + 3])); }
+    for (size_t p = 0; p < C + Z; p++) { ch.observe(F(open[4 * p + 2])); ch.observe(F(open[4 * p + 3])); }
   }
 
   E2 fri_alpha = ch.ext_challenge();
   {
     const u32 RW = S ? S->comm.world : 1;
     const u32 GS = RW > 1 ? (u32)SPLIT_BLOCK : 128;
-    std::vector<u64> wall;
-    auto plan = [&](u32 npoly, E2 weight0, u64 stride) { size_t off = wall.size(); u32 ng = (npoly + GS - 1) / GS; E2 ag = e2_pow(fri_alpha, stride), cur = weight0;
-                                                         for (u32 k = 0; k < ng; k++) { wall.push_back(cur.a.v); wall.push_back(cur.b.v); cur = cur * ag; } return off; };
+    size_t nw = 0;
+    bool w_over = false;
+    auto plan = [&](u32 npoly, E2 weight0, u64 stride) { size_t off = nw; u32 ng = (npoly + GS - 1) / GS; E2 ag = e2_pow(fri_alpha, stride), cur = weight0;
+                                                         for (u32 k = 0; k < ng; k++) { if (nw + 2 > 4096) { w_over = true; break; }
+                                                                                        P->h_w[nw++] = cur.a.v; P->h_w[nw++] = cur.b.v; cur = cur * ag; }
+                                                         return off; };
     const size_t tc0 = S ? (size_t)S->comm.rank * GS : 0, tcn = S ? S->cr : C, tzn = S ? S->zr : Z;
     const u64 gstride = (u64)GS * RW;
     size_t w_t = tcn ? plan((u32)tcn, e2_pow(fri_alpha, RW > 1 ? tc0 : 0), gstride) : 0, w_z = tzn ? plan((u32)tzn, e2_pow(fri_alpha, C + (RW > 1 ? tc0 : 0)), gstride) : 0,
            w_q = plan(4, e2_pow(fri_alpha, C + Z), GS);
-    if (wall.size() > 4096) return fail(SBN_ERR_UNSUPPORTED, "too many FRI combine groups");
-    HIPC(hipMemcpyAsync(P->d_w, wall.data(), wall.size() * sizeof(u64), hipMemcpyHostToDevice, st));
+    if (w_over) return fail(SBN_ERR_UNSUPPORTED, "too many FRI combine groups");
+    HIPC(hipMemcpyAsync(P->d_w, P->h_w, nw * sizeof(u64), hipMemcpyHostToDevice, st));
     hipLaunchKernelGGL(ext_pow_table_kernel, dim3(1), dim3(GS), 0, st, P->d_apow, P->d_apow + GS, (size_t)GS, fri_alpha.a.v, fri_alpha.b.v);
     auto combine = [&](const u64* coeffs, u32 npoly, size_t woff, u64* oa, u64* ob, int accumulate) -> int {
       u32 ng = (npoly + GS - 1) / GS;
@@ -1515,7 +1519,6 @@
     }
     HIPC(hipMemcpyAsync(f0a, f1a, 2 * n * sizeof(u64), hipMemcpyDeviceToDevice, st));
     if ((rc = combine(P->d_q, 4, w_q, f0a, f0b, 1))) return rc;
-    HIPC(stream_wait(st));
     HIPC(hipMemsetAsync(P->d_fcoef, 0, 2 * m * sizeof(u64), st));
     E2 shift2 = e2_pow(fri_alpha, C + Z);
     auto divide = [&](const u64* ca, const u64* cb, E2 z, E2 mul, int accumulate) {
@@ -1536,14 +1539,10 @@
     u32 bits = P->lde_log;
     u64* coef = P->d_fcoef; u64* coef_alt = P->d_fcoef2;
     size_t clen = m;
-    F shift(GL_GEN);
     for (size_t li = 0; li < P->fri.arity_bits.size(); li++) {
       u32 ab = P->fri.arity_bits[li];
       u64* va = P->fri_vals[li]; u64* vb = va + clen;
-      HIPC(hipMemcpyAsync(va, coef, 2 * clen * sizeof(u64), hipMemcpyDeviceToDevice, st));
-      hipLaunchKernelGGL(scale_pow_kernel, blocks(clen), dim3(256), 0, st, va, clen, shift.v);
-      hipLaunchKernelGGL(scale_pow_kernel, blocks(clen), dim3(256), 0, st, vb, clen, shift.v);
-      if ((rc = ntt_columns(P, va, clen, va, clen, P->d_tmp, m, 2, bits, false, clen, nullptr, nullptr, 1))) return rc;
+      if ((rc = ntt_columns(P, coef, clen, va, clen, P->d_tmp, m, 2, bits, false, clen, P->fri_shift[li], nullptr, 1))) return rc;
       DevTree& t = P->fri_trees[li];
       if (t.nleaf <= 16384) hipLaunchKernelGGL(fri_leaf_hash_coop_kernel, blocks(t.nleaf * 16), dim3(256), 0, st, va, vb, bits, ab, t.d);
       else hipLaunchKernelGGL(fri_leaf_hash_kernel, blocks(t.nleaf), dim3(256), 0, st, va, vb, bits, ab, t.d);
@@ -1558,13 +1557,12 @@
       HIPC(hipGetLastError());
       std::swap(coef, coef_alt);
       clen = nout; bits -= ab;
-      shift = f_pow(shift, (u64)1 << ab);
     }
     size_t fl = clen >> cfg.rate_bits;
     final_poly.resize(2 * fl);
-    std::vector<u64> fa(fl), fb(fl);
-    HIPC(hipMemcpyAsync(fa.data(), coef, fl * sizeof(u64), hipMemcpyDeviceToHost, st));
-    HIPC(hipMemcpyAsync(fb.data(), coef + clen, fl * sizeof(u64), hipMemcpyDeviceToHost, st));
+    const u64 *fa = P->h_xfer, *fb = P->h_xfer + fl;
+    HIPC(hipMemcpyAsync(P->h_xfer, coef, fl * sizeof(u64), hipMemcpyDeviceToHost, st));
+    HIPC(hipMemcpyAsync(P->h_xfer + fl, coef + clen, fl * sizeof(u64), hipMemcpyDeviceToHost, st));
     HIPC(stream_wait(st));
     for (size_t i = 0; i < fl; i++) { final_poly[2 * i] = fa[i]; final_poly[2 * i + 1] = fb[i]; ch.observe(F(fa[i])); ch.observe(F(fb[i])); }
   }
@@ -1579,12 +1577,12 @@
     for (int round = 0; pow_witness == ~0ULL; round++) {
       const u64 BATCH = round == 0 ? (1ULL << 17) : (1ULL << 20);
       if (base >= GLP - BATCH) return fail(SBN_ERR_HIP, "proof of work failed");
-      u64 init = ~0ULL;
-      HIPC(hipMemcpyAsync(P->d_pow, &init, sizeof(u64), hipMemcpyHostToDevice, st));
+      HIPC(hipMemsetAsync(P->d_pow, 0xFF, sizeof(u64), st));
       pp.base = base; pp.count = BATCH;
       hipLaunchKernelGGL(pow_kernel, blocks(BATCH), dim3(256), 0, st, pp);
-      HIPC(hipMemcpyAsync(&pow_witness, P->d_pow, sizeof(u64), hipMemcpyDeviceToHost, st));
+      HIPC(hipMemcpyAsync(P->h_xfer, P->d_pow, sizeof(u64), hipMemcpyDeviceToHost, st));
       HIPC(stream_wait(st));
+      pow_witness = P->h_xfer[0];
       base += BATCH;
     }
     ch.observe(F(pow_witness));
@@ -1663,9 +1661,9 @@
   if (Z) w.insert(w.end(), z_cap.begin(), z_cap.end());
   w.insert(w.end(), q_cap.begin(), q_cap.end());
   for (size_t p = 0; p < C; p++) { w.push_back(open[4 * p]); w.push_back(open[4 * p + 1]); }
-  for (size_t p = 0; p < C; p++) { w.push_back(open2[4 * p + 2]); w.push_back(open2[4 * p + 3]); }
+  for (size_t p = 0; p < C; p++) { w.push_back(open[4 * p + 2]); w.push_back(open[4 * p + 3]); }
   for (size_t p = C; p < C + Z; p++) { w.push_back(open[4 * p]); w.push_back(open[4 * p + 1]); }
-  for (size_t p = C; p < C + Z; p++) { w.push_back(open2[4 * p + 2]); w.push_back(open2[4 * p + 3]); }
+  for (size_t p = C; p < C + Z; p++) { w.push_back(open[4 * p + 2]); w.push_back(open[4 * p + 3]); }
   for (size_t p = C + Z; p < C + Z + 4; p++) { w.push_back(open[4 * p]); w.push_back(open[4 * p + 1]); }
   for (auto& cap : fri_caps) w.insert(w.end(), cap.begin(), cap.end());
   w.insert(w.end(), qwords.begin(), qwords.end());
```
